# Monash-Connected-Autonomous-Vehicle/unsupervised-pseuso-LiDAR

Hardware: AMD Instinct MI355X
Metric: images/sec (fwd+bwd) KITTI 192x640 triplets, full training step (higher is better)
Workload: dtype f32; 1 GPU; BASELINE.json configs[1]: per-GPU batch=12, 192x640 KITTI-shaped triplets, ResNet-18 depth encoder + 6-DoF PoseNet, fp32 (the ResNet trunk's 3x3 stride-1 convolutions and their data gradients: fp32 contractions on split operands -- three bf16 planes per operand, six bf16-MFMA plane products, fp32 accumulation; every other launch: fp32 MFMA), one step = 2x depth fwd + pose fwd + warp/L1/smooth loss; global_batch=12, parallelism=dp1

## Files before the change

include/mcav_conv.h:

```cpp
#ifndef MCAV_CONV_H
#define MCAV_CONV_H

#include <stddef.h>
#include <stdint.h>

#ifdef __cplusplus
extern "C" {
#endif

#define MCAV_G_DIRECT 0
#define MCAV_G_SMALLC 1
#define MCAV_G_ADJ_REFLECT 2
#define MCAV_G_ADJ_STRIDE2 3

#define MCAV_PAD_ZERO 0
#define MCAV_PAD_REFLECT 1

#define MCAV_ACT_NONE 0
#define MCAV_ACT_RELU 1
#define MCAV_ACT_ELU 2
#define MCAV_ACT_SIGMOID 3

#define MCAV_DACT_AFTER_ADDEND 0x100

typedef struct mcav_igemm_desc {
    const float* x1;
    const float* x2;
    int B, Hs, Ws, C1, C2;
    int up1;
    const float* w;
    int kh, kw, Np, Kp;
    int mode, stride, sign, offset, pad_mode;
    float* y;
    int Hd, Wd, Cd, n_begin, n_count, y_choff;
    const float* bias;
    int act;
    const float* dact_aux;
    int dact;
    const float* addend;
    int pool;
    float* stats;
    int tile;
    int groups;
    const float* w_upmerge;
    int mma;
    const void* w16;
    const float* stats_x;
    const float* stats_mean;
    const float* stats_invstd;
    const float* w_stem;
    const float* x_planar[3];
    int planar_B;
    int planar_stack;
} mcav_igemm_desc;

int mcav_igemm_mtiles(const mcav_igemm_desc* d);
int mcav_igemm(const mcav_igemm_desc* d, void* stream);
int mcav_igemm_uses_bf16(const mcav_igemm_desc* d);

typedef struct mcav_wgrad_desc {
    const float* x1;
    const float* x2;
    int B, Hs, Ws, C1, C2, up1;
    int kh, kw, Kp;
    int mode, stride, sign, offset, pad_mode;
    const float* dy;
    int Hd, Wd, Cdy, dy_choff;
    int Cout, Cin;
    float* dw_oihw;
    int accumulate;
    float* dbias;
    int tile;
    int upm, Cin_total, ci_offset;
    int mma;
    const float* dy_bn_x;
    const float* dy_bn_gamma;
    const float* dy_bn_mean;
    const float* dy_bn_invstd;
    const float* dy_bn_sums;
    int dy_bn_groups;
    float dy_bn_inv_count;
    const float* x_planar[3];
    int planar_B;
    int planar_stack;
} mcav_wgrad_desc;

size_t mcav_wgrad_workspace_bytes(const mcav_wgrad_desc* d);
int mcav_wgrad_uses_bf16(const mcav_wgrad_desc* d);
int mcav_wgrad(const mcav_wgrad_desc* d, void* workspace, size_t workspace_bytes, void* stream);

typedef struct mcav_wgrad_reduce_item {
    const float* slab;
    float* pre;
    float* dw;
    float* dbias;
    unsigned long long elems;
    int splits, groups, per_group, Ktot, slabN, Kp, taps, Cout, Cin, ci_t, accumulate, upm, cin_total, ci_off;
    int pre_bx, red_gx, red_gy, pre_first, red_first, reserved;
} mcav_wgrad_reduce_item;
int mcav_wgrad_deferred(const mcav_wgrad_desc* d, void* workspace, size_t workspace_bytes, mcav_wgrad_reduce_item* item, void* stream);
int mcav_wgrad_reduce_plan(mcav_wgrad_reduce_item* items, int n, int* presum_blocks, int* reduce_blocks, size_t* lds_bytes);
int mcav_wgrad_reduce_multi(const mcav_wgrad_reduce_item* items_dev, int n, int presum_blocks, int reduce_blocks, size_t lds_bytes, void* stream);

int mcav_pack_weights(const float* w_oihw, int Cout, int Cin, int kh, int kw, int transposed, float* packed, int Np, int Kp,
                      void* stream);

int mcav_pack_weights_multi(const void* items_dev, int nitems, int nblocks, void* stream);
int mcav_f32_to_bf16(const float* src, void* dst_bf16, size_t n, void* stream);
int mcav_f32_to_bf16_planes(const float* src, void* dst_bf16, size_t n, void* stream);
int mcav_pack_weights_blocks(int taps, int transposed, int Np, int Kp);
int mcav_pack_stem_weights(const float* w_oihw, int Cout, int Cin, float* packed, void* stream);
int mcav_pack_weights_upmerge(const float* w_oihw, int Cout, int Cin, int C1, float* packed, int Np, void* stream);
int mcav_pack_weights_upmerge_adj(const float* w_oihw, int Cout, int Cin, int C1, float* packed, int Np, int Kp, void* stream);
int mcav_upsample_adj_fold(const float* tmp, int B, int Hl, int Wl, int C, const float* dact_aux, int dact, const float* addend, float* out,
                           void* stream);

int mcav_conv3x3r_c1_fwd(const float* x, int B, int H, int W, int C, const float* w_oihw, const float* bias, int act, float* y,
                         void* stream);
size_t mcav_conv3x3r_c1_bwd_workspace_bytes(int C);
int mcav_conv3x3r_c1_bwd(const float* x, int B, int H, int W, int C, const float* w_oihw, const float* dy, const float* y, int act,
                         int x_act, const float* addend, float* dx, float* dw_oihw, float* dbias, int accumulate, void* workspace,
                         size_t workspace_bytes, void* stream);

int mcav_kernel_timer_begin(void);
int mcav_kernel_timer_count(void);
int mcav_kernel_timer_end(float* ms, int capacity);

int mcav_nchw_to_nhwc(const float* src, int B, int C, int H, int W, float* dst, int Cp, int choff, void* stream);
int mcav_nhwc_to_nchw(const float* src, int B, int C, int H, int W, int Cp, int choff, float* dst, void* stream);
int mcav_nchw3_to_nhwc(const float* s0, const float* s1, const float* s2, int B, int C, int H, int W, float* dst, int Cp, void* stream);

int mcav_bn_finalize(const float* stats, int mtiles, int C, double count, const float* gamma, const float* beta, float eps,
                     float momentum, float* running_mean, float* running_var, float* scale, float* shift, float* save_mean,
                     float* save_invstd, int groups, void* workspace, size_t workspace_bytes, void* stream);
size_t mcav_bn_finalize_workspace_bytes(int mtiles, int C, int groups);
int mcav_bn_eval_coeffs(const float* gamma, const float* beta, const float* running_mean, const float* running_var, float eps, int C,
                        float* scale, float* shift, void* stream);
int mcav_bn_apply(const float* x, const float* scale, const float* shift, const float* residual, int act, size_t n_pix, int C, float* y,
                  size_t pix_per_group, void* stream);
size_t mcav_bn_bwd_workspace_bytes(size_t n_pix, int C, int groups);
int mcav_bn_bwd_reduce(const float* dy, const float* y_act, const float* x, const float* save_mean, const float* save_invstd, int relu,
                       size_t n_pix, int C, float* dgamma, float* dbeta, int accumulate, float* sums ,
                       int groups, void* workspace, size_t workspace_bytes, void* stream);
int mcav_bn_bwd_finalize(const float* partial, int nblk, int C, float* dgamma, float* dbeta, int accumulate, float* sums, int groups, void* stream);
int mcav_bn_bwd_apply(const float* dy, const float* y_act, const float* x, const float* gamma, const float* save_mean,
                      const float* save_invstd, const float* sums, int relu, size_t n_pix, int C, float* dx, float* dres,
                      int dres_accumulate, int groups, void* stream);

int mcav_maxpool3s2_fwd(const float* x, int B, int H, int W, int C, float* y, uint8_t* idx, void* stream);
int mcav_maxpool3s2_bwd(const float* dy, const uint8_t* idx, int B, int H, int W, int C, float* dx, int accumulate, void* stream);

int mcav_stem_bn_relu_pool_fwd(const float* x, const float* scale, const float* shift, int B, int H, int W, int C, int groups, float* y,
                               float* pooled, uint8_t* idx, void* stream);
int mcav_stem_pool_bn_bwd_reduce(float* dy, const float* dpooled, const uint8_t* idx, const float* x, const float* scale, const float* shift,
                                 const float* save_mean, const float* save_invstd, int B, int H, int W, int C, int groups, int store_dz,
                                 float* dgamma, float* dbeta, int accumulate, float* sums , void* workspace,
                                 size_t workspace_bytes, void* stream);
int mcav_stem_pool_bn_bwd_apply(const float* dy, const float* dpooled, const uint8_t* idx, const float* x, const float* scale,
                                const float* shift, const float* gamma, const float* save_mean, const float* save_invstd, const float* sums,
                                int B, int H, int W, int C, int groups, float* dx, void* stream);

int mcav_act_bwd(const float* dy, const float* y, int act, size_t n, float* dx, int accumulate, void* stream);
int mcav_act_bwd_strided(const float* dy, const float* y, int act, size_t n, float* dx, int stride, void* stream);
int mcav_add(const float* a, const float* b, size_t n, float* out, void* stream);
int mcav_spatial_mean(const float* x, int B, int n_pix, int C, float scale, float* out, void* stream);
int mcav_spatial_mean_bwd(const float* dout, int B, int n_pix, int C, float scale, float* dx, void* stream);

int mcav_copy_channels(const float* src, size_t n_pix, int Cs, int soff, float* dst, int Cd, int doff, int C, int accumulate, void* stream);
int mcav_resize_bilinear_fwd(const float* src, int B, int h, int w, float* dst, int H, int W, float scale_y, float scale_x, void* stream);
int mcav_resize_bilinear_bwd(const float* ddst, int B, int h, int w, float* dsrc, int H, int W, float scale_y, float scale_x, int accumulate,
                             void* stream);
int mcav_upsample_nearest2x(const float* src, size_t planes, int h, int w, float* dst, void* stream);
int mcav_upsample_nearest2x_bwd(const float* grad_out, size_t planes, int h, int w, float* grad_in, void* stream);
int mcav_affine(const float* x, float a, float b, size_t n, float* y, void* stream);
int mcav_mul(const float* a, const float* b, size_t n, float* y, void* stream);
size_t mcav_colsum_workspace_bytes(int C);
int mcav_colsum(const float* x, size_t n_pix, int C, float* out, int accumulate, void* workspace, size_t workspace_bytes, void* stream);

int mcav_adam_step(float* param, const float* grad, float* exp_avg, float* exp_avg_sq, size_t n, float lr, float beta1, float beta2,
                   float eps, int step, float grad_scale, void* stream);

int mcav_adam_step_dev(float* param, const float* grad, float* exp_avg, float* exp_avg_sq, size_t n, float beta1, float beta2, float eps,
                       float* state8, void* stream);

int mcav_event_create(void** event);
int mcav_event_destroy(void* event);
int mcav_event_record_external(void* event, void* stream);
int mcav_event_wait_external(void* event, void* stream);
int mcav_stream_wait_event(void* stream, void* event);

#ifdef __cplusplus
}
#endif
#endif
```

unsupervised-pseuso-lidar_amd/csrc/conv_bf16.hip:

```cpp
#include "conv_shared.h"
#include "kernel_timer.h"

namespace mcav {

typedef __bf16 bf16x8 __attribute__((ext_vector_type(8)));
typedef __bf16 bf16x4 __attribute__((ext_vector_type(4)));
typedef __bf16 bf16x2 __attribute__((ext_vector_type(2)));
typedef unsigned short u16;
typedef unsigned int u32x2 __attribute__((ext_vector_type(2)));

template <int BM_, int BN_, int WM_, int WN_, int MF_, int CK_>
struct BTile {
    static constexpr int BM = BM_, BN = BN_, WM = WM_, WN = WN_, MF = MF_;
    static constexpr int KD = CK_;
    static constexpr int LDH = CK_ + 8;
    static constexpr int LPRA = CK_ / 4;
    static constexpr int RPPA = 256 / LPRA;
    static constexpr int AROWS = BM / RPPA;
    static constexpr int LPRB = CK_ / 8;
    static constexpr int BVECS = (BN * LPRB + 255) / 256;
    static constexpr int WAVES_M = BM / WM, WAVES_N = BN / WN;
    static constexpr int TM = WM / MF, TN = WN / MF;
    static constexpr int ACC = MF == 32 ? 16 : 4;
    using AccT = typename std::conditional<MF_ == 32, f32x16, f32x4>::type;
// ... 262 lines not shown
            issue(ra, rb, ex);
            store(ra, rb, ex, B0{});
            if (T_total > 1) issue(ra, rb, ex);
        }
    } else {
        if (T_total > 0) {
            issue(ra, rb, ex);
            if (T_total > 1) issue(ra2, rb2, ex2);
            store(ra, rb, ex, B0{});
            if (T_total > 2) issue(ra, rb, ex);
        }
    }
    __syncthreads();
    if constexpr (NS == 1) {
        int t = 0;
        for (; t + 1 < T_total; t += 2) {
            store(ra, rb, ex, B1{});
            if (t + 2 < T_total) issue(ra, rb, ex);
            compute(B0{});
            __syncthreads();
            if (t + 2 < T_total) {
                store(ra, rb, ex, B0{});
                if (t + 3 < T_total) issue(ra, rb, ex);
            }
            compute(B1{});
            __syncthreads();
        }
        if (t < T_total) {
            compute(B0{});
            __syncthreads();
        }
    } else {
        for (int t = 0; t < T_total; t += 2) {
            compute(B0{});
            __syncthreads();
            if (t + 1 < T_total) {
                store(ra2, rb2, ex2, B0{});
                if (t + 3 < T_total) issue(ra2, rb2, ex2);
                __syncthreads();
                compute(B0{});
                __syncthreads();
                if (t + 2 < T_total) {
                    store(ra, rb, ex, B0{});
                    if (t + 4 < T_total) issue(ra, rb, ex);
                    __syncthreads();
                }
            }
        }
#pragma unroll
        for (int i = 0; i < T::TM; ++i)
#pragma unroll
            for (int j = 0; j < T::TN; ++j) acc[i][j] += mid[i][j] + low[i][j];
    }
    igemm_epilogue_lean<T>(p, acc, s_out, s_stat, tid, wm0, wn0, n0, mt);
}

__device__ __forceinline__ int patch_pixel(int R) {
    const int r = R & 31;
    const bool g0 = r < 4 || (r >= 12 && r < 16) || (r >= 20 && r < 28);
    const int idx = g0 ? (r < 4 ? r : (r < 16 ? r - 8 : r - 12)) : (r < 12 ? r - 4 : (r < 20 ? r - 8 : r - 16));
    return (R & ~31) + (g0 ? 0 : 16) + idx;
}

__device__ __forceinline__ int small_div(int n, float rcp_d) { return (int)(((float)n + 0.5f) * rcp_d); }

struct PatchGeo {
    int TH, TW, tiles_y, tiles_x;
    int tmb;
    int refl;
};

#ifndef MCAV_PATCH_DIAG
#define MCAV_PATCH_DIAG 0
#endif

template <int TMB>
struct PatchCfg {
    static constexpr int BM = 64 * TMB;
    static constexpr int PIX = TMB == 1 ? 110 : 180;
    static constexpr int NJ = (PIX + 31) / 32;
    using T = typename std::conditional<TMB == 1, BT64x64k32, BT128x64k32>::type;
};

template <int NS, int TMB, bool ADJ = false>
__global__ __launch_bounds__(256, 2) void conv3x3_patch_kernel(IgemmParams p, const u16* __restrict__ w16, PatchGeo geo) {
    using C = PatchCfg<TMB>;
    using T = typename C::T;
    constexpr int BM = C::BM, BN = 64, CKT = 32, LDH = 32, PATCH_PIX = C::PIX;
    constexpr int APL = PATCH_PIX * LDH, BPL = BN * LDH;
    extern __shared__ __attribute__((aligned(16))) unsigned char s_raw[];
    u16* const Ap = reinterpret_cast<u16*>(s_raw);
    u16* const Bs = Ap + NS * APL;
    unsigned* const s_out = reinterpret_cast<unsigned*>(Bs + 3 * NS * BPL);
    float (*const s_stat)[2][BN] = reinterpret_cast<float (*)[2][BN]>(Bs);
    static_assert(sizeof(u16) * BPL >= sizeof(float) * T::WAVES_M * 2 * BN, "statistics scratch fits a filter plane");

    const int tid = threadIdx.x, lane = tid & 63, wave = tid >> 6;
    const int lid = xcd_remap(blockIdx.x, gridDim.x);
    const int nt = lid % p.ntiles, mt = lid / p.ntiles;
    const int n0 = nt * BN;
    const GatherSrc& g = p.g;
    const int TH = geo.TH, TW = geo.TW, PW = TW + 2, PH = TH + 2;
    const int per_img = geo.tiles_y * geo.tiles_x;
    const float rcp_pw = 1.0f / (float)PW, rcp_tw = 1.0f / (float)TW;
    const int img = small_div(mt, 1.0f / (float)per_img), tr = mt - img * per_img;
    const int tyi = small_div(tr, 1.0f / (float)geo.tiles_x);
    const int ty0 = tyi * TH, tx0 = (tr - tyi * geo.tiles_x) * TW;
// ... 176 lines not shown
                    mid[t] = __builtin_amdgcn_mfma_f32_32x32x16_bf16(a[0], b[1], mid[t], 0, 0, 0);
                    low[t] = __builtin_amdgcn_mfma_f32_32x32x16_bf16(a[1], b[1], low[t], 0, 0, 0);
                }
            }
            __builtin_amdgcn_sched_barrier(0);
        }
    };

    constexpr bool TWO = TMB == 1;
    f32x4 ra[C::NJ], rb0[3][NS], rb1[TWO ? 3 : 1][NS];
    const int total = nchunks * 3;
    issueA(ra, 0);
    issueB(rb0, 0);
    storeA(ra);
    storeB(rb0);
    if (total > 1) issueB(rb0, 1);
    if constexpr (TWO) {
        if (total > 2) issueB(rb1, 2);
    }
    __syncthreads();
    int ky = 0, chunk = 0;
    constexpr int diag = MCAV_PATCH_DIAG;
    auto stage = [&](int s, auto& rb_next) {
        const bool more = chunk + 1 < nchunks;
        if (ky == 0 && more && !(diag & 4)) issueA(ra, chunk + 1);
        if (!(diag & 8)) compute(ky);
        if constexpr (ADJ) {
            if (has_y1 | has_yl | has_x1 | has_xl) extras(ky);
        }
        if (!(diag & 2)) __syncthreads();
        if (ky == 2 && more && !(diag & 4)) storeA(ra);
        if (s + 1 < total) {
            if (!(diag & 1)) {
                storeB(rb_next);
                if (s + (TWO ? 3 : 2) < total) issueB(rb_next, s + (TWO ? 3 : 2));
            }
            if (!(diag & 2)) __syncthreads();
        }
        if (++ky == 3) { ky = 0; ++chunk; }
    };
    if constexpr (TWO) {
        for (int s = 0; s < total; s += 2) {
            stage(s, rb0);
            if (s + 1 < total) stage(s + 1, rb1);
        }
    } else {
        for (int s = 0; s < total; ++s) stage(s, rb0);
    }
    if constexpr (NS > 1) {
#pragma unroll
        for (int t = 0; t < TMB; ++t) acc[t][0] += mid[t] + low[t];
    }
    if (diag & 16) return;
    igemm_epilogue_lean<T>(p, acc, s_out, s_stat, tid, wm0, wn0, n0, mt);
}

template <int NS, int TMB>
constexpr size_t patch_lds_bytes() { return sizeof(u16) * (size_t)NS * (PatchCfg<TMB>::PIX + 3 * 64) * 32 + sizeof(unsigned) * 64 * TMB; }

struct P3Tile {
    static constexpr int BM = 192, BN = 64, MF = 32, ACC = 16, TM = 1, TN = 1, WAVES_M = 6, WAVES_N = 2;
    using AccT = f32x16;
};
constexpr int P3_THREADS = 768, P3_SUBS = 3, P3_PIX = 110;
template <int NS> constexpr size_t patch3_lds_bytes() { return sizeof(u16) * (size_t)NS * (P3_SUBS * P3_PIX + 2 * 3 * 64) * 32 + sizeof(unsigned) * 192; }
#ifndef MCAV_PATCH3_DIAG
#define MCAV_PATCH3_DIAG 0
#endif

template <int NS, bool ADJ>
__global__ __launch_bounds__(P3_THREADS, 1) void conv3x3_patch3_kernel(IgemmParams p, const u16* __restrict__ w16, PatchGeo geo) {
    using T = P3Tile;
    constexpr int BN = 64, CKT = 32, LDH = 32, PIX = P3_PIX;
    constexpr int APL = PIX * LDH, BPL = BN * LDH;
    constexpr int ASUB = NS * APL, BSTAGE = 3 * NS * BPL;
    constexpr int diag = MCAV_PATCH3_DIAG;
    extern __shared__ __attribute__((aligned(16))) unsigned char s_raw[];
    u16* const Ap = reinterpret_cast<u16*>(s_raw);
    u16* const Bs = Ap + P3_SUBS * ASUB;
    unsigned* const s_out = reinterpret_cast<unsigned*>(Bs + 2 * BSTAGE);
    float (*const s_stat)[2][BN] = reinterpret_cast<float (*)[2][BN]>(Bs);
    static_assert(sizeof(u16) * BSTAGE >= sizeof(float) * T::WAVES_M * 2 * BN, "statistics scratch fits a ring stage");

    const int tid = threadIdx.x, lane = tid & 63, wave = __builtin_amdgcn_readfirstlane(tid >> 6);
    const int sub = wave >> 2, wm0 = sub * 64 + ((wave >> 1) & 1) * 32, wn0 = (wave & 1) * 32;
    const int lid = xcd_remap(blockIdx.x, gridDim.x);
    const int nt = lid % p.ntiles, mt = lid / p.ntiles;
    const int n0 = nt * BN;
    const GatherSrc& g = p.g;
    const int TH = geo.TH, TW = geo.TW, PW = TW + 2, PH = TH + 2;
    const int per_img = geo.tiles_y * geo.tiles_x, nblocks = g.B * per_img;
    const float rcp_pw = 1.0f / (float)PW, rcp_tw = 1.0f / (float)TW;
    int b_img[P3_SUBS], b_ty0[P3_SUBS], b_tx0[P3_SUBS];
#pragma unroll
    for (int sb = 0; sb < P3_SUBS; ++sb) {
        const int blk = mt * P3_SUBS + sb;
        const int img = blk / per_img, tr = blk - img * per_img, tyi = tr / geo.tiles_x;
        b_img[sb] = blk < nblocks ? img : -1;
        b_ty0[sb] = tyi * TH;
        b_tx0[sb] = (tr - tyi * geo.tiles_x) * TW;
    }
    auto pick = [&](const int (&v)[P3_SUBS], int sb) { return sb == 0 ? v[0] : (sb == 1 ? v[1] : v[2]); };

    if (tid < 192) {
        const int sb = tid >> 6;
        const int pix = patch_pixel(tid & 63);
        const int py = small_div(pix, rcp_tw), px = pix - py * TW;
// ... 134 lines not shown
        const int rsh = (fwd ? ky : 2 - ky) * PW + (fwd ? 0 : 2);
        const int dxr = fwd ? 1 : -1;
        bf16x8 fa[2][NS], fb[2][NS];
        auto load = [&](int i, bf16x8 (&a)[NS], bf16x8 (&b)[NS]) {
            const int kx = i >> 1, ks = i & 1;
            const u16* const bp = Bst + (ks ? b_lane1 : b_lane0) + kx * NS * BPL;
#pragma unroll
            for (int q = 0; q < NS; ++q) b[q] = *reinterpret_cast<const bf16x8*>(bp + q * BPL);
            const int row = prow + rsh + kx * dxr;
            const u16* const ap = Asub + row * LDH + (((2 * ks + fslot) ^ ((row >> 2) & 3)) * 8);
#pragma unroll
            for (int q = 0; q < NS; ++q) a[q] = *reinterpret_cast<const bf16x8*>(ap + q * APL);
        };
        load(0, fa[0], fb[0]);
#pragma unroll
        for (int i = 0; i < 6; ++i) {
            if (i + 1 < 6) load(i + 1, fa[(i + 1) & 1], fb[(i + 1) & 1]);
            __builtin_amdgcn_sched_barrier(0);
            if (!(diag & 8)) mma(fa[i & 1], fb[i & 1]);
            __builtin_amdgcn_sched_barrier(0);
        }
    };

    f32x4 ra[NJ], rbn[NS];
    const int total = nchunks * 3;
    issueA(ra, 0);
    issueB(rbn, 0);
    storeA(ra);
    storeB(rbn, 0);
    if (total > 1) issueB(rbn, 1);
    __syncthreads();
    int ky = 0, chunk = 0;
    for (int s = 0; s < total; ++s) {
        const bool more = chunk + 1 < nchunks;
        const u16* const Bst = Bs + (s & 1) * BSTAGE;
        if (ky == 0 && more && !(diag & 4)) issueA(ra, chunk + 1);
        compute(ky, Bst);
        if constexpr (ADJ) {
            if (has_y1 | has_yl | has_x1 | has_xl) extras(ky, Bst);
        }
        if (s + 1 < total && !(diag & 1)) {
            storeB(rbn, (s + 1) & 1);
            if (s + 2 < total) issueB(rbn, s + 2);
        }
        if (ky == 2 && more && !(diag & 4)) {
            __syncthreads();
            storeA(ra);
        }
        __syncthreads();
        if (++ky == 3) { ky = 0; ++chunk; }
    }
    if constexpr (NS > 1) acc[0][0] += mid + low;
    if (diag & 16) return;
    igemm_epilogue_lean<T>(p, acc, s_out, s_stat, tid, wm0, wn0, n0, mt);
}

#ifndef MCAV_PATCH2_DIAG
#define MCAV_PATCH2_DIAG 0
#endif

template <int SB, int BN_>
struct Patch2Cfg {
    static constexpr int BM = 64 * SB, BN = BN_;
    static constexpr int PIX = 110;
    static constexpr int VP = SB * PIX;
    static constexpr int NJ = (VP + 31) / 32;
    using T = typename std::conditional<SB == 4, BTile<256, BN_, 64, BN_, 32, 32>, BTile<128, BN_, 32, BN_, 32, 32>>::type;
};

template <int NS, int SB, int BN>
constexpr size_t patch2_lds_bytes() { return sizeof(u16) * (size_t)NS * (SB * 110 + 2 * 3 * BN) * 32 + sizeof(unsigned) * 64 * SB; }

template <int NS, int SB, int BN>
__global__ __launch_bounds__(256, BN == 32 ? 2 : 1) void conv3x3_patch2_kernel(IgemmParams p, const u16* __restrict__ w16, PatchGeo geo) {
    using C = Patch2Cfg<SB, BN>;
    using T = typename C::T;
    constexpr int BM = C::BM, CKT = 32, LDH = 32, PIX = C::PIX, TM = T::TM, TN = T::TN;
    constexpr int APL = PIX * LDH;
    constexpr int BPL = BN * LDH;
    constexpr int BSTAGE = 3 * NS * BPL;
    extern __shared__ __attribute__((aligned(16))) unsigned char s_raw[];
    u16* const Ap = reinterpret_cast<u16*>(s_raw);
    u16* const Bs = Ap + SB * NS * APL;
    unsigned* const s_out = reinterpret_cast<unsigned*>(Bs + 2 * BSTAGE);
    float (*const s_stat)[2][BN] = reinterpret_cast<float (*)[2][BN]>(Bs);
    static_assert(sizeof(u16) * BSTAGE >= sizeof(float) * T::WAVES_M * 2 * BN, "statistics scratch fits a filter stage");

    const int tid = threadIdx.x, lane = tid & 63, wave = tid >> 6;
    const int lid = xcd_remap(blockIdx.x, gridDim.x);
    const int nt = lid % p.ntiles, mt = lid / p.ntiles;
    const int n0 = nt * BN;
    const GatherSrc& g = p.g;
    const int TH = geo.TH, TW = geo.TW, PW = TW + 2, PH = TH + 2;
    const int per_img = geo.tiles_y * geo.tiles_x, nblk = g.B * per_img;

    __shared__ int s_pp[C::PIX];
    if (tid < PIX) {
        const int ppy = tid / PW;
        s_pp[tid] = tid < PH * PW ? (ppy << 8) | (tid - ppy * PW) : -1;
    }
    int sb_base[SB], sb_y0[SB], sb_x0[SB];
#pragma unroll
    for (int sb = 0; sb < SB; ++sb) {
        const int blk = mt * SB + sb;
        const int img = blk / per_img, tr = blk - img * per_img, tyi = tr / geo.tiles_x;
        sb_base[sb] = blk < nblk ? img : -1;
        sb_y0[sb] = tyi * TH;
// ... 1300 lines not shown
```

unsupervised-pseuso-lidar_amd/csrc/conv_gather.h:

```cpp
#pragma once
#include "mcav_common.h"
#include "../../include/mcav_conv.h"

namespace mcav {

typedef float f32x4 __attribute__((ext_vector_type(4)));
typedef float f32x16 __attribute__((ext_vector_type(16)));

constexpr int CK = 16;
constexpr int LDK = CK + 4;

struct GatherSrc {
    const float* x1;
    const float* x2;
    int B, Hs, Ws, C1, C2, up1;
    int mode, stride, sign, offset, pad_mode;
};

__device__ __forceinline__ int reflect_idx(int i, int n) {
    i = i < 0 ? -i : i;
    return i >= n ? 2 * n - 2 - i : i;
}

__device__ __forceinline__ f32x4 load_src4(const GatherSrc& g, int n, int sy, int sx, int c) {
// ... 23 lines not shown

__device__ __forceinline__ f32x4 gather4(const GatherSrc& g, int n, int dy, int dx, int ky, int kx, int c) {
    f32x4 z = {0.f, 0.f, 0.f, 0.f};
    if (g.mode == MCAV_G_DIRECT || g.mode == MCAV_G_SMALLC) {
        int sy = dy * g.stride + g.sign * ky + g.offset;
        int sx = dx * g.stride + g.sign * kx + g.offset;
        if (g.pad_mode == MCAV_PAD_REFLECT) {
            sy = reflect_idx(sy, g.Hs);
            sx = reflect_idx(sx, g.Ws);
        } else if ((unsigned)sy >= (unsigned)g.Hs || (unsigned)sx >= (unsigned)g.Ws) {
            return z;
        }
        return load_src4(g, n, sy, sx, c);
    }
    if (g.mode == MCAV_G_ADJ_REFLECT) {
        int ys[2], xs[2], ny = 0, nx = 0;
        const int sy = dy + 1 - ky, sx = dx + 1 - kx;
        if ((unsigned)sy < (unsigned)g.Hs) ys[ny++] = sy;
        if (dy == 1 && ky == 0) ys[ny++] = 0;
        if (dy == g.Hs - 2 && ky == 2) ys[ny++] = g.Hs - 1;
        if ((unsigned)sx < (unsigned)g.Ws) xs[nx++] = sx;
        if (dx == 1 && kx == 0) xs[nx++] = 0;
        if (dx == g.Ws - 2 && kx == 2) xs[nx++] = g.Ws - 1;
        for (int a = 0; a < ny; ++a)
            for (int b = 0; b < nx; ++b) z += load_src4(g, n, ys[a], xs[b], c);
        return z;
    }
    const int ty = dy + g.offset - ky, tx = dx + g.offset - kx;
    if (ty < 0 || tx < 0 || ((ty | tx) & 1)) return z;
    const int sy = ty >> 1, sx = tx >> 1;
    if (sy >= g.Hs || sx >= g.Ws) return z;
    return load_src4(g, n, sy, sx, c);
}

__device__ __forceinline__ int xcd_remap(int bid, int nwg) {
    const int q = nwg >> 3, r = nwg & 7, xcd = bid & 7;
    return (xcd < r ? xcd * (q + 1) : r * (q + 1) + (xcd - r) * q) + (bid >> 3);
}

struct IgemmParams {
    GatherSrc g;
    const float* w;
    int kh, kw, Kp, Kstride, taps;
    float* y;
    int Hd, Wd, Cd, n_begin, n_count, y_choff;
    const float* bias;
    int act;
    const float* dact_aux;
    int dact;
    const float* addend;
    int pool;
    float* stats;
    const float *stats_x, *stats_mean, *stats_invstd;
    int M;
    int Mc, McP;
    int groups;
    int mtiles, ntiles;
    int no_tab;
    const float* wm;
    int Np_all;
    int bm;
    int upm;
    int ksplit;
    float* kslab;
};

__device__ __forceinline__ float act_fwd(float v, int act) {
    if (act == MCAV_ACT_RELU) return v > 0.f ? v : 0.f;
    if (act == MCAV_ACT_ELU) return v > 0.f ? v : expm1f(v);
    if (act == MCAV_ACT_SIGMOID) return 1.0f / (1.0f + expf(-v));
    return v;
}

__device__ __forceinline__ float act_bwd(float y, int act) {
    if (act == MCAV_ACT_RELU) return y > 0.f ? 1.f : 0.f;
    if (act == MCAV_ACT_ELU) return y > 0.f ? 1.f : y + 1.f;
    if (act == MCAV_ACT_SIGMOID) return y * (1.f - y);
    return 1.f;
}

typedef unsigned int u32x4 __attribute__((ext_vector_type(4)));
constexpr unsigned OOB = 0x80000000u;

__device__ __forceinline__ __amdgpu_buffer_rsrc_t make_rsrc(const void* ptr, unsigned bytes) {
    return __builtin_amdgcn_make_buffer_rsrc(const_cast<void*>(ptr), 0, bytes, 0x00020000);
}

__device__ __forceinline__ f32x4 buf_load4(__amdgpu_buffer_rsrc_t r, unsigned byte_off) {
    return __builtin_bit_cast(f32x4, __builtin_amdgcn_raw_buffer_load_b128(r, (int)byte_off, 0, 0));
}

__device__ __forceinline__ f32x4 buf_load4s(__amdgpu_buffer_rsrc_t r, unsigned byte_off, int sbyte_off) {
    return __builtin_bit_cast(f32x4, __builtin_amdgcn_raw_buffer_load_b128(r, (int)byte_off, sbyte_off, 0));
}

__device__ __forceinline__ float buf_load1(__amdgpu_buffer_rsrc_t r, unsigned byte_off) {
    return __builtin_bit_cast(float, __builtin_amdgcn_raw_buffer_load_b32(r, (int)byte_off, 0, 0));
}

__device__ __forceinline__ void buf_store1(__amdgpu_buffer_rsrc_t r, unsigned byte_off, float v) {
    __builtin_amdgcn_raw_buffer_store_b32(__builtin_bit_cast(unsigned, v), r, (int)byte_off, 0, 0);
}

}
```

unsupervised-pseuso-lidar_amd/csrc/conv_igemm.hip:

```cpp
#include <stdlib.h>
#include <map>
#include <mutex>
#include <type_traits>
#include <utility>

#include "conv_shared.h"
#include "kernel_timer.h"

namespace mcav {

template <class T, int KIND>
__global__ __launch_bounds__(256) void igemm_kernel(IgemmParams p) {
    constexpr int BM = T::BM, BN = T::BN;
    constexpr int CK = T::KD;
    __shared__ __attribute__((aligned(16))) float As[2][BM][T::LD];
    __shared__ __attribute__((aligned(16))) float Bs[2][BN][T::LD];
    __shared__ int s_out[BM];
    __shared__ float s_stat[T::WAVES_M][2][BN];
    constexpr int MAXTAB = 9;
    __shared__ unsigned s_o1[KIND == K_GENERIC ? 1 : MAXTAB][KIND == K_GENERIC ? 1 : BM];
    __shared__ unsigned s_o2[KIND == K_GENERIC ? 1 : MAXTAB][KIND == K_GENERIC ? 1 : BM];
    __shared__ int s_rn[KIND == K_GENERIC ? 1 : BM], s_ry[KIND == K_GENERIC ? 1 : BM], s_rx[KIND == K_GENERIC ? 1 : BM];

    const int tid = threadIdx.x, lane = tid & 63, wave = tid >> 6;
// ... 215 lines not shown
#pragma unroll
            for (int ks = 0; ks < CK / 8; ++ks) {
                f32x4 a[T::TM], b[T::TN];
#pragma unroll
                for (int i = 0; i < T::TM; ++i) a[i] = *reinterpret_cast<const f32x4*>(&As[buf][wm0 + i * 32 + frow][ks * 8 + fk]);
#pragma unroll
                for (int j = 0; j < T::TN; ++j) b[j] = *reinterpret_cast<const f32x4*>(&Bs[buf][wn0 + j * 32 + frow][ks * 8 + fk]);
#pragma unroll
                for (int q = 0; q < 4; ++q)
#pragma unroll
                    for (int i = 0; i < T::TM; ++i)
#pragma unroll
                        for (int j = 0; j < T::TN; ++j)
                            acc[i][j] = __builtin_amdgcn_mfma_f32_32x32x2f32(a[i][q], b[j][q], acc[i][j], 0, 0, 0);
            }
        } else {
            const int frow = lane & 15, fk = (lane >> 4) * 4;
#pragma unroll
            for (int ks = 0; ks < CK / 16; ++ks) {
                f32x4 a[T::TM], b[T::TN];
#pragma unroll
                for (int i = 0; i < T::TM; ++i) a[i] = *reinterpret_cast<const f32x4*>(&As[buf][wm0 + i * 16 + frow][ks * 16 + fk]);
#pragma unroll
                for (int j = 0; j < T::TN; ++j) b[j] = *reinterpret_cast<const f32x4*>(&Bs[buf][wn0 + j * 16 + frow][ks * 16 + fk]);
#pragma unroll
                for (int q = 0; q < 4; ++q)
#pragma unroll
                    for (int i = 0; i < T::TM; ++i)
#pragma unroll
                        for (int j = 0; j < T::TN; ++j)
                            acc[i][j] = __builtin_amdgcn_mfma_f32_16x16x4f32(a[i][q], b[j][q], acc[i][j], 0, 0, 0);
            }
        }
    };

    f32x4 ra[T::AROWS], rb[T::BVECS];
    if (T_total > 0) {
        load_tile(ra, rb, true);
        store_tile(ra, rb, 0);
        if (T_total > 1) { advance(); load_tile(ra, rb, true); }
    }
    __syncthreads();
    for (int t = 0; t < T_total; ++t) {
        const int buf = t & 1;
        if (t + 1 < T_total) {
            store_tile(ra, rb, buf ^ 1);
            if (t + 2 < T_total) { advance(); load_tile(ra, rb, true); }
        }
        __builtin_amdgcn_sched_barrier(0);
        compute(buf);
        __builtin_amdgcn_sched_barrier(0);
        __syncthreads();
    }
    igemm_epilogue<T>(p, acc, s_out, s_stat, tid, wm0, wn0, n0, mt);
}


#ifndef MCAV_DIAG
#define MCAV_DIAG 0
#endif
#if MCAV_DIAG == 4
__device__ unsigned long long g_diag_stamps[8];
#define MCAV_STAMP_BEGIN() unsigned long long st_prev = __builtin_readcyclecounter()
#define MCAV_STAMP(i) do { __syncthreads(); if (threadIdx.x == 0) { const unsigned long long st_now = __builtin_readcyclecounter(); \
        atomicAdd(&g_diag_stamps[i], st_now - st_prev); if (i == 5) atomicAdd(&g_diag_stamps[0], 1ull); st_prev = st_now; } } while (0)
#else
#define MCAV_STAMP_BEGIN()
#define MCAV_STAMP(i)
#endif
#ifndef MCAV_IG_OCC
#define MCAV_IG_OCC 1
#endif
template <class T, int TK>
__global__ __launch_bounds__(256, (T::BM == 128 && T::BN == 64 && T::KD == 16 && TK != 1) ? 4
                                  : ((T::BM == 64 && T::BN == 64 && T::KD == 32 && TK == 0) ? MCAV_IG_OCC : 1)) void igemm_tab_kernel(IgemmParams p) {
    constexpr bool REFL = TK == 1, UPM = TK == 2;
    constexpr int BM = T::BM, BN = T::BN, CKT = T::KD;
    __shared__ __attribute__((aligned(16))) float As[2][BM][T::LD];
    __shared__ __attribute__((aligned(16))) float Bs[2][BN][T::LD];
    __shared__ __attribute__((aligned(16))) unsigned s_out[BM];
    float (*const s_stat)[2][BN] = reinterpret_cast<float (*)[2][BN]>(&As[1][0][0]);
    static_assert(sizeof(float) * BM * T::LD >= sizeof(float) * T::WAVES_M * 2 * BN, "statistics scratch fits one A buffer");
    extern __shared__ unsigned s_dyn[];
    unsigned* const s_o1 = s_dyn;
    unsigned* const s_o2 = s_dyn + (UPM ? 4 * BM : (p.g.C2 > 0 ? p.taps * BM : 0));
    int* const s_rn = reinterpret_cast<int*>(&As[0][0][0]);
    unsigned* const s_e0 = s_dyn + p.taps * BM;
    unsigned* const s_e1 = s_dyn + 2 * p.taps * BM;
    unsigned* const s_e2 = s_dyn + 3 * p.taps * BM;
    int* const s_ry = s_rn + BM;
    int* const s_rx = s_rn + 2 * BM;
    static_assert(2 * BM * T::LD >= 3 * BM, "row coordinates fit the A panel");
    __shared__ int s_tl[TAB_TAPS + 1];
    __shared__ int s_nt;

    const int tid = threadIdx.x, lane = tid & 63, wave = tid >> 6;
    MCAV_STAMP_BEGIN();
    const int lid = p.g.mode == MCAV_G_ADJ_STRIDE2 ? (int)blockIdx.x : xcd_remap(blockIdx.x, gridDim.x);
    const int per_split = p.mtiles * p.ntiles;
    const int ks = p.ksplit > 1 ? lid / per_split : 0, lrem = lid - ks * per_split;
    const int nt = lrem % p.ntiles, mt = lrem / p.ntiles;
    const int m0 = mt * BM, n0 = nt * BN;
    const GatherSrc& g = p.g;

    for (int r = tid; r < (MCAV_DIAG >= 5 ? 0 : BM); r += 256) {
        int n, dy, dx;
        const bool ok = decode_row(p, m0 + r, n, dy, dx);
// ... 363 lines not shown
                    else if constexpr (WHOLE_ISSUE && P == T::AROWS + T::BVECS) issue(ra, rb);
                    else piece(std::integral_constant<int, P>{}, nxt);
                });
                __builtin_amdgcn_sched_barrier(0);
            });
        });
        if constexpr (MCAV_DIAG < 3) __syncthreads();
    };
    MCAV_STAMP(1);
    int t = 0;
    using Yes = std::true_type;
    using No = std::false_type;
    if (T_total > 0) {
        if constexpr (REFL) {
            issue(ra, rb);
            store(ra, rb, B0{});
            if (T_total > 1) issue(ra, rb);
        } else if constexpr (MCAV_DIAG >= 6) {
#pragma unroll
            for (int j = 0; j < T::AROWS; ++j) ra[j] = f32x4{1.f, 1.f, 1.f, 1.f};
#pragma unroll
            for (int j = 0; j < T::BVECS; ++j) rb[j] = f32x4{1.f, 1.f, 1.f, 1.f};
            store(ra, rb, B0{});
        } else {
            f32x4 ra0[T::AROWS], rb0[T::BVECS];
            issue(ra0, rb0);
            if (T_total > 1) issue(ra, rb);
            store(ra0, rb0, B0{});
        }
    }
    __syncthreads();
    MCAV_STAMP(2);
    for (; t + 3 < T_total; t += 2) {
        step(B0{}, B1{}, Yes{}, Yes{});
        step(B1{}, B0{}, Yes{}, Yes{});
    }
    MCAV_STAMP(3);
    const int rest = T_total - t;
    if (rest == 3) {
        step(B0{}, B1{}, Yes{}, Yes{});
        step(B1{}, B0{}, Yes{}, No{});
        step(B0{}, B1{}, No{}, No{});
    } else if (rest == 2) {
        step(B0{}, B1{}, Yes{}, No{});
        step(B1{}, B0{}, No{}, No{});
    } else if (rest == 1) {
        step(B0{}, B1{}, No{}, No{});
    }
    MCAV_STAMP(4);
    if (p.ksplit > 1) {
        IgemmParams q = p;
        q.y = p.kslab + (size_t)ks * ((size_t)p.g.B * p.Hd * p.Wd * p.Cd);
        q.bias = nullptr; q.act = MCAV_ACT_NONE; q.dact_aux = nullptr; q.addend = nullptr; q.stats = nullptr; q.stats_x = nullptr;
        igemm_epilogue_lean<T>(q, acc, s_out, s_stat, tid, wm0, wn0, n0, mt);
    } else {
        igemm_epilogue_lean<T>(p, acc, s_out, s_stat, tid, wm0, wn0, n0, mt);
    }
    MCAV_STAMP(5);
}

template <class T, int KIND>
__global__ __launch_bounds__(256) void wgrad_kernel(WgradParams p) {
    constexpr int BM = T::BM, BN = T::BN;
    __shared__ __attribute__((aligned(16))) float Xs[2][KP][BM];
    __shared__ __attribute__((aligned(16))) float Ys[2][KP][BN];
    const int tid = threadIdx.x, lane = tid & 63, wave = tid >> 6;
    const int per_split = p.mtiles * p.ntiles;
    const int lid_ = xcd_remap(blockIdx.x, gridDim.x);
    const int split = lid_ / per_split, rem = lid_ - split * per_split;
    const int nt = rem % p.ntiles, mt = rem / p.ntiles;
    const int m0 = mt * BM, n0 = nt * BN;
    const GatherSrc& g = p.g;

    constexpr int ACOLS = BM / 4;
    constexpr int APIX = 256 / ACOLS;
    constexpr int APASS = KP / APIX;
    constexpr int CPW = ACOLS / 4;
    const int acol = wave * CPW + lane % CPW, apix = lane / CPW;
    const int kflat = m0 + acol * 4;
    int aky = -1, akx = 0, ac = 0;
    if (kflat < p.Ktot) {
        const int tap = kflat / p.Kp;
        ac = kflat - tap * p.Kp;
        aky = tap / p.kw; akx = tap - aky * p.kw;
        if (tap >= p.taps) aky = -1;
    }
    constexpr int BCOLS = BN / 4;
    constexpr int BPIX = 256 / BCOLS > KP ? KP : 256 / BCOLS;
    constexpr int BPASS = KP / BPIX;
    const int bcol = tid % BCOLS, bpix = tid / BCOLS;

    const int pix_begin = split * p.pix_per_split;
    const int pix_end = min(p.Mpix, pix_begin + p.pix_per_split);
    const int T_total = pix_end > pix_begin ? (pix_end - pix_begin + KP - 1) / KP : 0;

    int pn, py, px;
    {
        const int m = pix_begin + apix;
        pn = m / (p.Hd * p.Wd);
        const int r = m - pn * (p.Hd * p.Wd);
        py = r / p.Wd; px = r - py * p.Wd;
    }
    auto step_pix = [&](int& n, int& y, int& x, int by) {
        x += by;
        if constexpr (KIND == K_FAST) {
            const bool wx = x >= p.Wd;
            x = wx ? x - p.Wd : x;
            y += wx ? 1 : 0;
            const bool wy = y >= p.Hd;
// ... 786 lines not shown
inline int kstride_of(int taps, int Kp) { return round_up(taps * Kp, CK); }

inline int pick_tile(const mcav_igemm_desc* d, long M) {
    if (d->tile) return d->tile;
    if (d->n_count <= 16) return (M >= 256 * 64 && d->kh * d->kw <= 16) ? 4 : 6;
    if (d->n_count <= 32) return 7;
    if (d->mode == MCAV_G_ADJ_REFLECT && ((M + 127) / 128) * ((d->n_count + 63) / 64) >= 1024) return 2;
    if (d->mode != MCAV_G_SMALLC && ((M + 127) / 128) * ((d->n_count + 63) / 64) >= 1024) return 1;
    const long t64 = ((M + 63) / 64) * ((d->n_count + 63) / 64);
    if (d->mode != MCAV_G_SMALLC && d->Kp % 32 == 0 && (t64 <= 128 || (t64 > 256 && t64 < 512))) return 12;
    if (d->mode != MCAV_G_SMALLC && d->Kp % 32 == 0) return 10;
    const long t128x64 = ((M + 127) / 128) * ((d->n_count + 63) / 64);
    return t128x64 >= 1024 ? 1 : 2;
}

void tile_dims(int id, int& BM, int& BN) {
    switch (id) {
        case 1: BM = 128; BN = 64; break;
        case 2: BM = 64; BN = 64; break;
        case 3: BM = 256; BN = 32; break;
        case 4: BM = 256; BN = 16; break;
        case 5: BM = 128; BN = 128; break;
        case 7: BM = 128; BN = 32; break;
        case 8: BM = 128; BN = 64; break;
        case 9: BM = 128; BN = 128; break;
        case 10: BM = 64; BN = 64; break;
        case 11: BM = 64; BN = 64; break;
        case 12: BM = 32; BN = 64; break;
        default: BM = 64; BN = 16; break;
    }
}

bool fill_params(const mcav_igemm_desc* d, IgemmParams& p, int& tile) {
    if (!d || !d->x1 || !d->w || !d->y) return false;
    if (d->B <= 0 || d->Hs <= 0 || d->Ws <= 0 || d->Hd <= 0 || d->Wd <= 0 || d->C1 <= 0 || d->C2 < 0) return false;
    if (d->C2 > 0 && !d->x2) return false;
    if (d->kh <= 0 || d->kw <= 0 || d->Np <= 0 || d->Kp <= 0 || d->kh * d->kw > 64) return false;
    if (d->n_begin < 0 || d->n_count <= 0 || d->n_begin + d->n_count > d->Np) return false;
    if (d->mode == MCAV_G_SMALLC) { if (d->Kp != 4 || d->C1 != 4 || d->C2 != 0) return false; }
    else if (d->Kp % CK != 0 || d->Kp < d->C1 + d->C2) return false;
    if (d->C2 > 0 && (d->C1 % 4 != 0)) return false;
    if (d->mode == MCAV_G_ADJ_REFLECT && (d->kh != 3 || d->kw != 3 || d->Hs != d->Hd || d->Ws != d->Wd || d->Hs < 2 || d->Ws < 2)) return false;
    if (d->pad_mode == MCAV_PAD_REFLECT && (d->Hs < 2 || d->Ws < 2)) return false;
    if (d->up1 && ((d->Hs & 1) || (d->Ws & 1))) return false;
    if (d->pool && ((d->Hd & 1) || (d->Wd & 1) || d->mode == MCAV_G_ADJ_STRIDE2)) return false;
    if (d->pool && d->stats) return false;
    p.g.x1 = d->x1; p.g.x2 = d->x2; p.g.B = d->B; p.g.Hs = d->Hs; p.g.Ws = d->Ws; p.g.C1 = d->C1; p.g.C2 = d->C2; p.g.up1 = d->up1;
    p.g.mode = d->mode; p.g.stride = d->stride; p.g.sign = d->sign; p.g.offset = d->offset; p.g.pad_mode = d->pad_mode;
    p.w = d->w; p.kh = d->kh; p.kw = d->kw; p.Kp = d->Kp; p.taps = d->kh * d->kw; p.Kstride = kstride_of(p.taps, d->Kp);
    p.y = d->y; p.Hd = d->Hd; p.Wd = d->Wd; p.Cd = d->Cd; p.n_begin = d->n_begin; p.n_count = d->n_count; p.y_choff = d->y_choff;
    p.bias = d->bias; p.act = d->act; p.dact_aux = d->dact_aux; p.dact = d->dact; p.addend = d->addend; p.pool = d->pool; p.stats = d->stats;
    if (d->stats_x && (!d->stats || !d->stats_mean || !d->stats_invstd || d->pool || d->y_choff != 0 || d->n_begin != 0 || d->n_count != d->Cd)) return false;
    p.stats_x = d->stats ? d->stats_x : nullptr; p.stats_mean = d->stats_mean; p.stats_invstd = d->stats_invstd;
    const long Mlin = (long)d->B * d->Hd * d->Wd;
    if ((long)d->B * d->Hs * d->Ws * (d->C1 > d->C2 ? d->C1 : d->C2) * 4 >= 0x7fffffffL) return false;
    if ((long)d->Np * kstride_of(d->kh * d->kw, d->Kp) * 4 >= 0x7fffffffL) return false;
    p.no_tab = (d->tile >> 8) & 1;
    p.ksplit = 1; p.kslab = nullptr;
    p.wm = d->w_upmerge; p.Np_all = d->Np; p.upm = 0;
    tile = pick_tile(d, Mlin) & 0xff;
    if (tile == 0) { mcav_igemm_desc dd = *d; dd.tile = 0; tile = pick_tile(&dd, Mlin); }
    if (((tile >= 8 && tile <= 10) || tile == 12) && (d->mode == MCAV_G_SMALLC || d->Kp % 32 != 0)) return false;
    if (tile == 11 && (d->mode == MCAV_G_SMALLC || d->Kp % 64 != 0)) return false;
    int BM, BN;
    tile_dims(tile, BM, BN);
    p.groups = d->groups > 1 ? d->groups : 1;
    if (p.groups > 1) {
        if ((d->mode != MCAV_G_DIRECT && d->mode != MCAV_G_SMALLC) || d->pool || d->B % p.groups != 0) return false;
        p.Mc = (int)(Mlin / p.groups);
        p.McP = round_up(p.Mc, BM);
        p.M = p.groups * p.McP;
    } else if (d->mode == MCAV_G_ADJ_STRIDE2) {
        p.Mc = d->B * ((d->Hd + 1) / 2) * ((d->Wd + 1) / 2);
        p.McP = round_up(p.Mc, BM);
        p.M = 4 * p.McP;
    } else {
        p.Mc = 0; p.McP = 1;
        if (Mlin > 0x7fffffffL) return false;
        p.M = (int)Mlin;
        const int ck = (tile >= 8 && tile <= 10) || tile == 12 ? 32 : (tile == 11 ? 64 : 16);
        if (d->w_upmerge && d->mode == MCAV_G_DIRECT && d->kh == 3 && d->kw == 3 && d->stride == 1 && d->sign == 1 && d->offset == -1 &&
            d->pad_mode == MCAV_PAD_REFLECT && d->up1 == 1 && d->C2 > 0 && !(d->Hd & 1) && !(d->Wd & 1) && d->Hd == d->Hs && d->Wd == d->Ws &&
            !d->pool && !d->stats && d->C1 % ck == 0 && d->C2 % ck == 0 && d->C1 + d->C2 == d->Kp && (d->C1 & 3) == 0 && !p.no_tab &&
            (long)4 * d->Np * 4 * d->C1 * 4 < 0x7fffffffL) {
            p.upm = 1;
            p.bm = BM;
            p.Mc = d->B * (d->Hd / 2) * (d->Wd / 2);
            p.McP = round_up(p.Mc, BM);
            p.M = 4 * p.McP;
        }
    }
    p.mtiles = (p.M + BM - 1) / BM;
    p.ntiles = (d->n_count + BN - 1) / BN;
    return true;
}

__global__ __launch_bounds__(256) void splitk_finish_kernel(const float* __restrict__ slab, int splits, size_t n, int Cd, float* __restrict__ y,
                                                            const float* __restrict__ bias, int n_begin, int act, const float* __restrict__ dact_aux,
                                                            int dact, const float* __restrict__ addend) {
    for (size_t i = (size_t)blockIdx.x * 256 + threadIdx.x; i < n; i += (size_t)gridDim.x * 256) {
        float v = 0.f;
        for (int k = 0; k < splits; ++k) v += slab[(size_t)k * n + i];
        if (bias) v += bias[n_begin + (int)(i % (size_t)Cd)];
        v = act_fwd(v, act);
        if (dact_aux && !(dact & MCAV_DACT_AFTER_ADDEND)) v *= act_bwd(dact_aux[i], dact & 0xff);
        if (addend) v += addend[i];
// ... 41 lines not shown
            if (ksp > 8) ksp = 8;
            if (ksp > ktiles / 4) ksp = ktiles / 4;
            if (ksp >= 2) {
                float* slab = ksplit_slab(s, (size_t)p.g.B * p.Hd * p.Wd * p.Cd * 4 * ksp);
                if (slab) { p.ksplit = ksp; p.kslab = slab; }
            }
        }
    }
    const int grid = p.mtiles * p.ntiles * p.ksplit;
    const size_t tab_bytes = sizeof(unsigned) * (size_t)p.taps * T::BM * (p.g.C2 > 0 ? 2 : 1);
    const size_t refl_bytes = sizeof(unsigned) * (size_t)p.taps * T::BM * 4;
    if (p.upm) timed_launch(igemm_tab_kernel<T, 2>, grid, dim3(256), sizeof(unsigned) * 13 * T::BM, s, p);
    else if (tab) timed_launch(igemm_tab_kernel<T, 0>, grid, dim3(256), tab_bytes, s, p);
    else if (tab_refl) timed_launch(igemm_tab_kernel<T, 1>, grid, dim3(256), refl_bytes, s, p);
    else if (fast_mode && c4ok) timed_launch(igemm_kernel<T, K_FAST>, grid, dim3(256), 0, s, p);
    else if (p.g.mode == MCAV_G_ADJ_REFLECT && c4ok && p.g.C2 == 0) timed_launch(igemm_kernel<T, K_REFLADJ>, grid, dim3(256), 0, s, p);
    else timed_launch(igemm_kernel<T, K_GENERIC>, grid, dim3(256), 0, s, p);
    if (p.ksplit > 1) {
        const size_t n = (size_t)p.g.B * p.Hd * p.Wd * p.Cd;
        const int blocks = (int)((n + 255) / 256 < 2048 ? (n + 255) / 256 : 2048);
        timed_launch(splitk_finish_kernel, blocks, dim3(256), 0, s, (const float*)p.kslab, p.ksplit, n, p.Cd, p.y, p.bias, p.n_begin, p.act, p.dact_aux,
                     p.dact, p.addend);
    }
}

}

using namespace mcav;

int mcav_bf16_igemm_mtiles(const mcav_igemm_desc* d);
int mcav_patch_f32_mtiles(const mcav_igemm_desc* d);
bool mcav_try_patch_f32(const mcav_igemm_desc* d, hipStream_t s);
int mcav_stem_mtiles(const mcav_igemm_desc* d);

int mcav_stem_planar_igemm(const mcav_igemm_desc* d);

MCAV_EXPORT int mcav_igemm_mtiles(const mcav_igemm_desc* d) {
    IgemmParams p;
    int tile;
    const int planar = mcav_stem_planar_igemm(d);
    if (planar < 0) return MCAV_E_INVALID;
    mcav_igemm_desc dp;
    if (planar) { dp = *d; if (!dp.x1) dp.x1 = d->x_planar[0]; d = &dp; }
    if (!fill_params(d, p, tile)) return MCAV_E_INVALID;
    if (const int st = mcav_stem_mtiles(d)) return st;
    if (const int pt = mcav_patch_f32_mtiles(d)) return pt;
    if (d->mma != 0) {
        const int mt = mcav_bf16_igemm_mtiles(d);
        if (mt > 0) return mt;
    }
    return p.mtiles;
}

bool mcav_try_halo(const mcav_igemm_desc* d, hipStream_t s);
int mcav_bf16_igemm(const mcav_igemm_desc* d, hipStream_t s);
bool mcav_try_stem(const mcav_igemm_desc* d, const mcav::IgemmParams& p, hipStream_t s);
int mcav_stem_mtiles(const mcav_igemm_desc* d);
int mcav_stem_planar_igemm(const mcav_igemm_desc* d);
bool mcav_bf16_wgrad_plan(const mcav_wgrad_desc* d, mcav::WgradPlan& pl);
void mcav_bf16_wgrad_launch(const mcav::WgradParams& p, hipStream_t s);

MCAV_EXPORT int mcav_igemm(const mcav_igemm_desc* d, void* stream) {
    IgemmParams p;
    int tile;
    const int planar = mcav_stem_planar_igemm(d);
    if (planar < 0) return MCAV_E_INVALID;
    mcav_igemm_desc dp;
    if (planar) { dp = *d; if (!dp.x1) dp.x1 = d->x_planar[0]; d = &dp; }
    if (!fill_params(d, p, tile)) return MCAV_E_INVALID;
    hipStream_t s = as_stream(stream);
    if (planar) return mcav_try_stem(d, p, s) ? launch_status() : MCAV_E_INVALID;
    if (mcav_try_halo(d, s)) return launch_status();
    if (mcav_try_stem(d, p, s)) return launch_status();
    if (mcav_try_patch_f32(d, s)) return launch_status();
    if (d->mma != 0) {
        const int rc = mcav_bf16_igemm(d, s);
        if (rc != 1) return rc;
    }
    switch (tile) {
        case 1: launch_igemm<Tile128x64>(p, s); break;
        case 2: launch_igemm<Tile64x64>(p, s); break;
        case 3: launch_igemm<Tile256x32>(p, s); break;
        case 4: launch_igemm<Tile256x16>(p, s); break;
        case 5: launch_igemm<Tile128x128>(p, s); break;
        case 6: launch_igemm<Tile64x16>(p, s); break;
        case 7: launch_igemm<Tile128x32>(p, s); break;
        case 8: launch_igemm<Tile128x64k32>(p, s); break;
        case 9: launch_igemm<Tile128x128k32>(p, s); break;
        case 10: launch_igemm<Tile64x64k32>(p, s); break;
        case 11: launch_igemm<Tile64x64k64>(p, s); break;
        case 12: launch_igemm<Tile32x64k32>(p, s); break;
        default: return MCAV_E_INVALID;
    }
    return launch_status();
}

namespace mcav {

}
int mcav_stem_wgrad_splits(const mcav_wgrad_desc* d);
int mcav_stem_planar_wgrad(const mcav_wgrad_desc* d);
int mcav_stem_wgrad_bn(const mcav_wgrad_desc* d);
void mcav_stem_wgrad_launch(const mcav_wgrad_desc* d, float* slab, int Ktot, int slabN, int splits, hipStream_t s);
int mcav_halo_wgrad_splits(const mcav_wgrad_desc* d);
void mcav_halo_wgrad_launch(const mcav_wgrad_desc* d, float* slab, int slabN, int splits, hipStream_t s);
namespace mcav {

bool plan_wgrad(const mcav_wgrad_desc* d, WgradPlan& pl) {
    if (!d || !d->x1 || !d->dy || !d->dw_oihw) return false;
    if (d->B <= 0 || d->Hs <= 0 || d->Ws <= 0 || d->Hd <= 0 || d->Wd <= 0 || d->C1 <= 0 || d->C2 < 0 || d->Cout <= 0 || d->Cin <= 0) return false;
    if (d->C2 > 0 && (!d->x2 || d->C1 % 4 != 0)) return false;
    if (d->mode != MCAV_G_DIRECT && d->mode != MCAV_G_SMALLC) return false;
    if (d->mode == MCAV_G_SMALLC && (d->Kp != 4 || d->C1 != 4 || d->C2 != 0)) return false;
    if (d->mode == MCAV_G_DIRECT && (d->Kp % CK != 0 || d->Kp < d->C1 + d->C2)) return false;
    if (d->Cin > d->Kp) return false;
    WgradParams& p = pl.p;
    p.g.x1 = d->x1; p.g.x2 = d->x2; p.g.B = d->B; p.g.Hs = d->Hs; p.g.Ws = d->Ws; p.g.C1 = d->C1; p.g.C2 = d->C2; p.g.up1 = d->up1;
    p.g.mode = d->mode; p.g.stride = d->stride; p.g.sign = d->sign; p.g.offset = d->offset; p.g.pad_mode = d->pad_mode;
    p.kh = d->kh; p.kw = d->kw; p.Kp = d->Kp; p.taps = d->kh * d->kw; p.Ktot = p.taps * d->Kp;
    p.dy = d->dy; p.Hd = d->Hd; p.Wd = d->Wd; p.Cdy = d->Cdy; p.dy_choff = d->dy_choff; p.Cout = d->Cout;
    p.CoutLoad = round_up(d->Cout, 4) <= d->Cdy - d->dy_choff ? round_up(d->Cout, 4) : d->Cout;
    const long M = (long)d->B * d->Hd * d->Wd;
    if (M > 0x7fffffffL) return false;
// ... 295 lines not shown
```

unsupervised-pseuso-lidar_amd/csrc/conv_shared.h:

```cpp
#pragma once
#include <stdlib.h>
#include <type_traits>
#include <utility>

#include "conv_gather.h"

namespace mcav {

template <int BM_, int BN_, int WM_, int WN_, int MF_, int CK_ = 16>
struct Tile {
    static constexpr int BM = BM_, BN = BN_, WM = WM_, WN = WN_, MF = MF_;
    static constexpr int KD = CK_;
    static constexpr int LD = CK_ + 4;
    static constexpr int LPR = CK_ / 4;
    static constexpr int RPP = 256 / LPR;
    static constexpr int WAVES_M = BM / WM, WAVES_N = BN / WN;
    static constexpr int TM = WM / MF, TN = WN / MF;
    static constexpr int ACC = MF == 32 ? 16 : 4;
    using AccT = typename std::conditional<MF_ == 32, f32x16, f32x4>::type;
    static constexpr int AROWS = BM / RPP;
    static constexpr int BVECS = (BN * LPR + 255) / 256;
    static_assert(WAVES_M * WAVES_N == 4, "4 wavefronts per workgroup");
    static_assert(BM % RPP == 0, "BM multiple of the rows per pass");
};
// ... 18 lines not shown

__device__ __forceinline__ bool decode_row(const IgemmParams& p, int m, int& n, int& dy, int& dx) {
    if (p.g.mode == MCAV_G_ADJ_STRIDE2) {
        const int blk = m / p.McP, r = m - blk * p.McP, cls = 3 - blk;
        if (r >= p.Mc) return false;
        const int Hc = (p.Hd + 1) >> 1, Wc = (p.Wd + 1) >> 1;
        n = r / (Hc * Wc);
        const int q = r - n * (Hc * Wc);
        const int y2 = q / Wc, x2 = q - y2 * Wc;
        dy = 2 * y2 + (cls >> 1);
        dx = 2 * x2 + (cls & 1);
        return dy < p.Hd && dx < p.Wd;
    }
    if (m >= p.M) return false;
    if (p.upm) {
        const int blk = m / p.bm, cls = blk & 3, r = (blk >> 2) * p.bm + (m - blk * p.bm);
        if (r >= p.Mc) return false;
        const int Hc = p.Hd >> 1, Wc = p.Wd >> 1;
        n = r / (Hc * Wc);
        const int q = r - n * (Hc * Wc);
        const int y2 = q / Wc, x2 = q - y2 * Wc;
        dy = 2 * y2 + (cls >> 1);
        dx = 2 * x2 + (cls & 1);
        return true;
    }
    if (p.groups > 1) {
        const int grp = m / p.McP, r = m - grp * p.McP;
        if (r >= p.Mc) return false;
        const int hw = p.Hd * p.Wd, ng = r / hw, q = r - ng * hw;
        n = grp * (p.g.B / p.groups) + ng;
        dy = q / p.Wd;
        dx = q - dy * p.Wd;
        return true;
    }
    if (p.pool) {
        const int blk = m >> 2, q = m & 3;
        const int Hh = p.Hd >> 1, Wh = p.Wd >> 1;
        n = blk / (Hh * Wh);
        const int r = blk - n * (Hh * Wh);
        const int y2 = r / Wh, x2 = r - y2 * Wh;
        dy = 2 * y2 + (q >> 1);
        dx = 2 * x2 + (q & 1);
        return true;
    }
    n = m / (p.Hd * p.Wd);
    const int r = m - n * (p.Hd * p.Wd);
    dy = r / p.Wd;
    dx = r - dy * p.Wd;
    return true;
}

enum { K_FAST = 0, K_REFLADJ = 1, K_GENERIC = 2 };

template <class T>
__device__ __forceinline__ void igemm_epilogue(const IgemmParams& p, typename T::AccT (&acc)[T::TM][T::TN], const int* s_out,
                                               float (*s_stat)[2][T::BN], int tid, int wm0, int wn0, int n0, int mt) {
    constexpr int BN = T::BN;
    const int lane = tid & 63, wave = tid >> 6;
    constexpr int MF = T::MF;
    const int ccol = lane & (MF - 1);
    float ssum[T::TN], ssq[T::TN];
#pragma unroll
    for (int j = 0; j < T::TN; ++j) { ssum[j] = 0.f; ssq[j] = 0.f; }
#pragma unroll
    for (int i = 0; i < T::TM; ++i)
#pragma unroll
        for (int j = 0; j < T::TN; ++j) {
            const int nl = n0 + wn0 + j * MF + ccol;
            const bool ncol = nl < p.n_count;
            const float bv = (p.bias && ncol) ? p.bias[p.n_begin + nl] : 0.f;
#pragma unroll
            for (int q = 0; q < T::ACC / 4; ++q) {
                const int rbase = wm0 + i * MF + (MF == 32 ? 8 * q + 4 * (lane >> 5) : 4 * (lane >> 4));
                float v[4];
#pragma unroll
                for (int e = 0; e < 4; ++e) v[e] = act_fwd(acc[i][j][4 * q + e] + bv, p.act);
                if (p.pool) {
                    const int o = s_out[rbase];
                    if (o >= 0 && ncol) {
                        float s = (v[0] + v[1]) + (v[2] + v[3]);
                        const size_t off = (size_t)o * p.Cd + p.y_choff + nl;
                        if (p.dact_aux && !(p.dact & MCAV_DACT_AFTER_ADDEND)) s *= act_bwd(p.dact_aux[off], p.dact & 0xff);
                        if (p.addend) s += p.addend[off];
                        if (p.dact_aux && (p.dact & MCAV_DACT_AFTER_ADDEND)) s *= act_bwd(p.dact_aux[off], p.dact & 0xff);
                        p.y[off] = s;
                    }
                } else {
#pragma unroll
                    for (int e = 0; e < 4; ++e) {
                        const int o = s_out[rbase + e];
                        if (o >= 0 && ncol) {
                            float s = v[e];
                            const size_t off = (size_t)o * p.Cd + p.y_choff + nl;
                            if (p.dact_aux && !(p.dact & MCAV_DACT_AFTER_ADDEND)) s *= act_bwd(p.dact_aux[off], p.dact & 0xff);
                            if (p.addend) s += p.addend[off];
                            if (p.dact_aux && (p.dact & MCAV_DACT_AFTER_ADDEND)) s *= act_bwd(p.dact_aux[off], p.dact & 0xff);
                            p.y[off] = s;
                            ssum[j] += s;
                            if (p.stats_x) {
                                const int gi = (mt / (p.mtiles / p.groups)) * p.n_count + nl;
                                ssq[j] += s * ((p.stats_x[off] - p.stats_mean[gi]) * p.stats_invstd[gi]);
                            } else {
                                ssq[j] += s * s;
                            }
                        }
                    }
                }
            }
        }
    if (p.stats) {
#pragma unroll
        for (int j = 0; j < T::TN; ++j) {
            if (MF == 32) {
                ssum[j] += __shfl_xor(ssum[j], 32, 64);
                ssq[j] += __shfl_xor(ssq[j], 32, 64);
            } else {
                ssum[j] += __shfl_xor(ssum[j], 16, 64); ssq[j] += __shfl_xor(ssq[j], 16, 64);
                ssum[j] += __shfl_xor(ssum[j], 32, 64); ssq[j] += __shfl_xor(ssq[j], 32, 64);
            }
            if (lane < MF) {
                s_stat[wave / T::WAVES_N][0][wn0 + j * MF + lane] = ssum[j];
                s_stat[wave / T::WAVES_N][1][wn0 + j * MF + lane] = ssq[j];
            }
        }
        __syncthreads();
        for (int e = tid; e < 2 * BN; e += 256) {
            const int which = e / BN, col = e - which * BN;
            if (n0 + col < p.n_count) {
                float s = 0.f;
#pragma unroll
                for (int wmi = 0; wmi < T::WAVES_M; ++wmi) s += s_stat[wmi][which][col];
                p.stats[((size_t)mt * 2 + which) * p.n_count + n0 + col] = s;
            }
        }
    }
}

template <class T>
__device__ __forceinline__ void igemm_epilogue_lean(const IgemmParams& p, typename T::AccT (&acc)[T::TM][T::TN], const unsigned* s_outb,
                                                    float (*s_stat)[2][T::BN], int tid, int wm0, int wn0, int n0, int mt) {
    constexpr int BN = T::BN, MF = T::MF, NQ = T::ACC / 4;
    const int lane = tid & 63, wave = tid >> 6;
    const int ccol = lane & (MF - 1);
    const unsigned ybytes = (unsigned)((size_t)p.g.B * (p.pool ? (p.Hd >> 1) * (p.Wd >> 1) : p.Hd * p.Wd) * p.Cd * 4);
    const __amdgpu_buffer_rsrc_t ry = make_rsrc(p.y, ybytes);
    const __amdgpu_buffer_rsrc_t rx = make_rsrc(p.dact_aux ? p.dact_aux : p.y, ybytes);
    const __amdgpu_buffer_rsrc_t rad = make_rsrc(p.addend ? p.addend : p.y, ybytes);
    const __amdgpu_buffer_rsrc_t rsx = make_rsrc(p.stats_x ? p.stats_x : p.y, ybytes);
    const int sgrp = p.stats_x ? (mt / (p.mtiles / p.groups)) * p.n_count : 0;
    float ssum[T::TN], ssq[T::TN];
#pragma unroll
    for (int j = 0; j < T::TN; ++j) { ssum[j] = 0.f; ssq[j] = 0.f; }
#pragma unroll
    for (int i = 0; i < T::TM; ++i)
#pragma unroll
        for (int j = 0; j < T::TN; ++j) {
            __builtin_amdgcn_sched_barrier(0);
            const int nl = n0 + wn0 + j * MF + ccol;
            if (nl < p.n_count) {
                const float bv = p.bias ? p.bias[p.n_begin + nl] : 0.f;
                const unsigned colb = (unsigned)(p.y_choff + nl) * 4u;
                u32x4 ro[NQ];
#pragma unroll
                for (int q = 0; q < NQ; ++q) {
                    const int rbase = wm0 + i * MF + (MF == 32 ? 8 * q + 4 * (lane >> 5) : 4 * (lane >> 4));
                    ro[q] = *reinterpret_cast<const u32x4*>(&s_outb[rbase]);
                }
                if (p.pool) {
                    float aux[NQ], add[NQ];
                    if (p.dact_aux) {
#pragma unroll
                        for (int q = 0; q < NQ; ++q) aux[q] = buf_load1(rx, ro[q].x + colb);
                    }
                    if (p.addend) {
#pragma unroll
                        for (int q = 0; q < NQ; ++q) add[q] = buf_load1(rad, ro[q].x + colb);
                    }
#pragma unroll
                    for (int q = 0; q < NQ; ++q) {
                        float v[4];
#pragma unroll
                        for (int e = 0; e < 4; ++e) v[e] = act_fwd(acc[i][j][4 * q + e] + bv, p.act);
                        float s = (v[0] + v[1]) + (v[2] + v[3]);
                        if (p.dact_aux && !(p.dact & MCAV_DACT_AFTER_ADDEND)) s *= act_bwd(aux[q], p.dact & 0xff);
                        if (p.addend) s += add[q];
                        if (p.dact_aux && (p.dact & MCAV_DACT_AFTER_ADDEND)) s *= act_bwd(aux[q], p.dact & 0xff);
                        buf_store1(ry, ro[q].x + colb, s);
                    }
                } else {
                    constexpr int QH = NQ >= 2 ? NQ / 2 : 1;
#pragma unroll
// ... 14 lines not shown
#pragma unroll
                                for (int e = 0; e < 4; ++e) aux[4 * q + e] = buf_load1(rx, ro[q0 + q][e] + colb);
                        }
                        if (p.addend) {
#pragma unroll
                            for (int q = 0; q < QH; ++q)
#pragma unroll
                                for (int e = 0; e < 4; ++e) add[4 * q + e] = buf_load1(rad, ro[q0 + q][e] + colb);
                        }
#pragma unroll
                        for (int q = 0; q < QH; ++q)
#pragma unroll
                            for (int e = 0; e < 4; ++e) {
                                float s = acc[i][j][4 * (q0 + q) + e] + bv;
                                if (p.act == MCAV_ACT_RELU) s = fmaxf(s, 0.f);
                                else if (p.act != MCAV_ACT_NONE) s = act_fwd(s, p.act);
                                if (p.dact_aux && !(p.dact & MCAV_DACT_AFTER_ADDEND)) s *= act_bwd(aux[4 * q + e], p.dact & 0xff);
                                if (p.addend) s += add[4 * q + e];
                                if (p.dact_aux && (p.dact & MCAV_DACT_AFTER_ADDEND)) s *= act_bwd(aux[4 * q + e], p.dact & 0xff);
                                buf_store1(ry, ro[q0 + q][e] + colb, s);
                                if (p.stats) {
                                    const float sv = ro[q0 + q][e] != OOB ? s : 0.f;
                                    ssum[j] += sv;
                                    ssq[j] += p.stats_x ? sv * ((xs[4 * q + e] - smu) * sis) : sv * sv;
                                }
                            }
                        __builtin_amdgcn_sched_barrier(0);
                    }
                }
            }
        }
    if (p.stats) {
#pragma unroll
        for (int j = 0; j < T::TN; ++j) {
            if (MF == 32) {
                ssum[j] += __shfl_xor(ssum[j], 32, 64);
                ssq[j] += __shfl_xor(ssq[j], 32, 64);
            } else {
                ssum[j] += __shfl_xor(ssum[j], 16, 64); ssq[j] += __shfl_xor(ssq[j], 16, 64);
                ssum[j] += __shfl_xor(ssum[j], 32, 64); ssq[j] += __shfl_xor(ssq[j], 32, 64);
            }
            if (lane < MF) {
                s_stat[wave / T::WAVES_N][0][wn0 + j * MF + lane] = ssum[j];
                s_stat[wave / T::WAVES_N][1][wn0 + j * MF + lane] = ssq[j];
            }
        }
        __syncthreads();
        for (int e = tid; e < 2 * BN; e += 256) {
            const int which = e / BN, col = e - which * BN;
            if (n0 + col < p.n_count) {
                float s = 0.f;
#pragma unroll
                for (int wmi = 0; wmi < T::WAVES_M; ++wmi) s += s_stat[wmi][which][col];
                p.stats[((size_t)mt * 2 + which) * p.n_count + n0 + col] = s;
            }
        }
    }
}

constexpr int TAB_TAPS = 32;
constexpr int WG_TABCAP = 2048;

struct WgradParams {
    GatherSrc g;
    int kh, kw, Kp, taps, Ktot;
    const float* dy;
    int Hd, Wd, Cdy, dy_choff, Cout;
    int CoutLoad;
    int Mpix;
    int splits, pix_per_split;
    int mtiles, ntiles;
    float* slab;
    int slabN;
    int want_bias;
    int tab_cht_log2;
    int upm;
    int Hf, Wf;
    int split_planes;
    int patch, pTH, pTW, ptiles_y, ptiles_x, prefl, pnblocks, pbps, pct_co, pnarrow;
};

constexpr int KP = 32;

struct WgradPlan {
    WgradParams p;
    int tile;
    bool use_tab;
    bool use_halo;
    bool use_stem;
    size_t slab_bytes, pre_bytes;
    int ci_t, groups, per_group;
};


bool fill_params(const mcav_igemm_desc* d, IgemmParams& p, int& tile);
bool plan_wgrad(const mcav_wgrad_desc* d, WgradPlan& pl);
void tile_dims(int id, int& BM, int& BN);

}
```

unsupervised-pseuso-lidar_amd/csrc/conv_stem.hip:

```cpp
#include "conv_shared.h"
#include "bn_bwd_formula.h"
#include "kernel_timer.h"

namespace mcav {

constexpr int ST_TW = 32;
constexpr int ST_PC = 36;

template <int C_, int CP_, int N_, int TH_>
struct StemCfg {
    static constexpr int C = C_, CP = CP_, N = N_, TH = TH_;
    static constexpr int PR = 2 * TH + 5;
    static constexpr int KS = C * 7 * 4;
    static constexpr int TM = TH / 4, TN = N >= 32 ? N / 32 : 1;
    static constexpr int NW = N;
    static constexpr int LD4 = (C + 3) / 4;
    using Epi = Tile<TH * 32, (N >= 32 ? N : 32), TM * 32, (N >= 32 ? N : 32), 32, 16>;
};
using StemDepth = StemCfg<3, 4, 64, 8>;
using StemPose = StemCfg<9, 16, 16, 4>;

struct StemPlanar {
    const float* src[3];
    int Bp;
// ... 162 lines not shown
    issue(blockIdx.x);
    for (int mt = blockIdx.x; mt < ntiles; mt += gridDim.x) {
        const int b = mt / per_img, tr = mt - b * per_img;
        const int ty = tr / tiles_x, tx = tr - ty * tiles_x;
        const int oy0 = ty * TH, ox0 = tx * ST_TW;
        __syncthreads();
        if (tid < TH * 32) {
            const int r = tid, oy = oy0 + (r >> 5), ox = ox0 + (r & 31);
            s_out[r] = (oy < p.Hd && ox < p.Wd) ? (unsigned)((b * p.Hd + oy) * p.Wd + ox) * (unsigned)(p.Cd * 4) : OOB;
        }
#pragma unroll
        for (int j = 0; j < PN; ++j) {
            const int i = tid + 256 * j;
            const int row = i / (2 * ST_PC), col = i - row * (2 * ST_PC);
            if (i < PR * 2 * ST_PC) {
#pragma unroll
                for (int c = 0; c < C; ++c) {
                    if constexpr (kPlanar) sP[c][row][col & 1][col >> 1] = pq[j][c];
                    else sP[c][row][col & 1][col >> 1] = pv[j][c >> 2][c & 3];
                }
            }
        }
        __syncthreads();
        issue(mt + gridDim.x);

        f32x16 acc[TM][TN];
#pragma unroll
        for (int i = 0; i < TM; ++i)
#pragma unroll
            for (int j = 0; j < TN; ++j)
#pragma unroll
                for (int r = 0; r < 16; ++r) acc[i][j][r] = 0.f;
        float fa[2][TM], fb[2][TN];
        auto rd = [&](auto sc) {
            constexpr int ks = decltype(sc)::value, kxp = ks & 3, cky = ks >> 2, ky = cky % 7, c = cky / 7, sl = ks & 1;
#pragma unroll
            for (int i = 0; i < TM; ++i) fa[sl][i] = pa[(c * PR + ky + 2 * i) * 2 * ST_PC + kxp];
#pragma unroll
            for (int j = 0; j < TN; ++j) fb[sl][j] = pb[ks * 2 * NW + 32 * j];
        };
        rd(std::integral_constant<int, 0>{});
        static_for<KS>([&](auto sc) {
            constexpr int ks = decltype(sc)::value, sl = ks & 1;
            if constexpr (ks + 1 < KS) rd(std::integral_constant<int, ks + 1>{});
            __builtin_amdgcn_sched_barrier(0);
#pragma unroll
            for (int i = 0; i < TM; ++i)
#pragma unroll
                for (int j = 0; j < TN; ++j) acc[i][j] = __builtin_amdgcn_mfma_f32_32x32x2f32(fa[sl][i], fb[sl][j], acc[i][j], 0, 0, 0);
            __builtin_amdgcn_sched_barrier(0);
        });
        __syncthreads();
        if constexpr (kWide) stem_epilogue_wide<E>(p, acc, s_out, s_stat, tid, wave * TM * 32, mt);
        else igemm_epilogue_lean<E>(p, acc, s_out, s_stat, tid, wave * TM * 32, 0, 0, mt);
    }
}

typedef __bf16 st_bf16x8 __attribute__((ext_vector_type(8)));
typedef __bf16 st_bf16x4 __attribute__((ext_vector_type(4)));
typedef unsigned short st_u16;
typedef unsigned int st_u32x2 __attribute__((ext_vector_type(2)));
constexpr int SS_TH = 8, SS_PR = 2 * SS_TH + 5, SS_PCOL = 72, SS_PROW = SS_PCOL * 4;
constexpr int SS_K = 224, SS_WROW = 232;
constexpr int SS_PPL = SS_PR * SS_PROW, SS_WPL = 64 * SS_WROW;
#ifndef MCAV_SS_DIAG
#define MCAV_SS_DIAG 0
#endif
constexpr int SS_DIAG = MCAV_SS_DIAG;
constexpr size_t stem_split_lds_bytes() { return sizeof(st_u16) * 3 * (size_t)(SS_PPL + SS_WPL) + sizeof(unsigned) * SS_TH * 32; }

__device__ __forceinline__ void st_split3(f32x4 v, st_u32x2& h, st_u32x2& m, st_u32x2& l) {
    const st_bf16x4 hb = __builtin_convertvector(v, st_bf16x4);
    const f32x4 r1 = v - __builtin_convertvector(hb, f32x4);
    const st_bf16x4 mb = __builtin_convertvector(r1, st_bf16x4);
    const f32x4 r2 = r1 - __builtin_convertvector(mb, f32x4);
    const st_bf16x4 lb = __builtin_convertvector(r2, st_bf16x4);
    h = __builtin_bit_cast(st_u32x2, hb); m = __builtin_bit_cast(st_u32x2, mb); l = __builtin_bit_cast(st_u32x2, lb);
}

template <bool kPlanar = false>
__global__ __launch_bounds__(256, 1) void stem7x7s2_split_fwd_kernel(IgemmParams p, const float* __restrict__ wk, int tiles_x, int tiles_y, StemPlanar pl) {
    using S = StemDepth;
    using E = typename S::Epi;
    constexpr int TM = S::TM, TN = S::TN, TH = S::TH;
    static_assert(TH == SS_TH && TM == 2 && TN == 2, "8 output rows per tile, 2 x 2 tiles per wavefront");
    extern __shared__ __attribute__((aligned(16))) unsigned char s_raw[];
    st_u16* const sP = reinterpret_cast<st_u16*>(s_raw);
    st_u16* const sW = sP + 3 * SS_PPL;
    unsigned* const s_out = reinterpret_cast<unsigned*>(sW + 3 * SS_WPL);
    float (*const s_stat)[2][E::BN] = reinterpret_cast<float (*)[2][E::BN]>(sP);

    const int tid = threadIdx.x, lane = tid & 63, wave = tid >> 6;
    const int per_img = tiles_x * tiles_y, ntiles = p.g.B * per_img;
    const GatherSrc& g = p.g;
    const __amdgpu_buffer_rsrc_t rsx = make_rsrc(g.x1, (unsigned)((size_t)g.B * g.Hs * g.Ws * S::CP * 4));

    constexpr int WN = 64 * SS_K / 256;
    float wv[WN];
#pragma unroll
    for (int j = 0; j < WN; ++j) {
        const int e = tid + 256 * j, co = e & 63, k = e >> 6, ky = k >> 5, kx = (k >> 2) & 7, c = k & 3;
        wv[j] = c < 3 ? wk[((c * 7 + ky) * 8 + kx) * 64 + co] : 0.f;
    }
#pragma unroll
    for (int j = 0; j < WN; ++j) {
        const int e = tid + 256 * j, co = e & 63, k = e >> 6;
        const float v = wv[j];
// ... 49 lines not shown
                *reinterpret_cast<st_u32x2*>(sP + i * 4) = hh;
                *reinterpret_cast<st_u32x2*>(sP + SS_PPL + i * 4) = mm;
                *reinterpret_cast<st_u32x2*>(sP + 2 * SS_PPL + i * 4) = ll;
            }
        }
        __syncthreads();
        issue(mt + gridDim.x);

        f32x16 acc[TM][TN], mid[TM][TN], low[TM][TN];
#pragma unroll
        for (int i = 0; i < TM; ++i)
#pragma unroll
            for (int j = 0; j < TN; ++j)
#pragma unroll
                for (int r = 0; r < 16; ++r) { acc[i][j][r] = 0.f; mid[i][j][r] = 0.f; low[i][j][r] = 0.f; }
        st_bf16x8 fa[2][TM][3], fb[2][TN][3];
        auto rd = [&](auto sc) {
            constexpr int ks = decltype(sc)::value, ky = ks >> 1, kh = ks & 1, sl = ks & 1;
#pragma unroll
            for (int i = 0; i < TM; ++i)
#pragma unroll
                for (int q = 0; q < 3; ++q) fa[sl][i][q] = *reinterpret_cast<const st_bf16x8*>(pa + q * SS_PPL + (2 * i + ky) * SS_PROW + 16 * kh);
#pragma unroll
            for (int j = 0; j < TN; ++j)
#pragma unroll
                for (int q = 0; q < 3; ++q) fb[sl][j][q] = *reinterpret_cast<const st_bf16x8*>(pb + q * SS_WPL + 32 * j * SS_WROW + 32 * ky + 16 * kh);
        };
        rd(std::integral_constant<int, 0>{});
        static_for<14>([&](auto sc) {
            constexpr int ks = decltype(sc)::value, sl = ks & 1;
            if constexpr (ks + 1 < 14) rd(std::integral_constant<int, ks + 1>{});
            __builtin_amdgcn_sched_barrier(0);
#pragma unroll
            for (int i = 0; i < TM; ++i)
#pragma unroll
                for (int j = 0; j < TN; ++j) {
                    const st_bf16x8(&a)[3] = fa[sl][i];
                    const st_bf16x8(&bq)[3] = fb[sl][j];
                    if (SS_DIAG & 1) continue;
                    low[i][j] = __builtin_amdgcn_mfma_f32_32x32x16_bf16(a[2], bq[0], low[i][j], 0, 0, 0);
                    mid[i][j] = __builtin_amdgcn_mfma_f32_32x32x16_bf16(a[1], bq[0], mid[i][j], 0, 0, 0);
                    acc[i][j] = __builtin_amdgcn_mfma_f32_32x32x16_bf16(a[0], bq[0], acc[i][j], 0, 0, 0);
                    low[i][j] = __builtin_amdgcn_mfma_f32_32x32x16_bf16(a[0], bq[2], low[i][j], 0, 0, 0);
                    mid[i][j] = __builtin_amdgcn_mfma_f32_32x32x16_bf16(a[0], bq[1], mid[i][j], 0, 0, 0);
                    low[i][j] = __builtin_amdgcn_mfma_f32_32x32x16_bf16(a[1], bq[1], low[i][j], 0, 0, 0);
                }
            __builtin_amdgcn_sched_barrier(0);
        });
#pragma unroll
        for (int i = 0; i < TM; ++i)
#pragma unroll
            for (int j = 0; j < TN; ++j) acc[i][j] += mid[i][j] + low[i][j];
        __syncthreads();
        if (!(SS_DIAG & 2)) igemm_epilogue_lean<E>(p, acc, s_out, s_stat, tid, wave * TM * 32, 0, 0, mt);
    }
}

__global__ void pack_stem_weights_kernel(const float* __restrict__ w, float* __restrict__ out, int C, int N) {
    const int i = blockIdx.x * blockDim.x + threadIdx.x;
    if (i >= C * 56 * N) return;
    const int n = i % N, k = i / N;
    const int hh = k & 1, j = (k >> 1) & 3, cky = k >> 3, ky = cky % 7, c = cky / 7;
    const int kx = 2 * j + hh;
    out[i] = kx < 7 ? w[((n * C + c) * 7 + ky) * 7 + kx] : 0.f;
}

constexpr int SW_TH = 4;
constexpr int SW_PR = 2 * SW_TH + 5;

struct StemWgradBn {
    const float* x;
    const float* gamma;
    const float* mean;
    const float* invstd;
    const float* sums;
    int groups;
    float inv_count;
};

template <int C, int CP, int N, int KP, bool kBN = false, bool kPlanar = false>
__global__ __launch_bounds__(256) void stem7x7s2_wgrad_kernel(const float* __restrict__ x4, const float* __restrict__ dy, int B, int Hs, int Ws,
                                                              int Hd, int Wd, int Cdy, int dy_choff, float* __restrict__ slab, int Ktot, int slabN,
                                                              int want_bias, StemWgradBn bn, StemPlanar pl) {
    constexpr int KS = C * 7 * 4, KT = (2 * KS + 31) / 32;
    constexpr int NSPLIT = N >= 64 ? 2 : 1, WPN = 4 / NSPLIT, MT = (KT + WPN - 1) / WPN;
    constexpr int LD4 = (C + 3) / 4, N4 = N / 4;
    __shared__ __attribute__((aligned(16))) float sP[C][SW_PR][2][ST_PC];
    __shared__ __attribute__((aligned(16))) float sDY[SW_TH * ST_TW][N];
    const int tid = threadIdx.x, lane = tid & 63, wave = tid >> 6;
    const int tiles_x = (Wd + ST_TW - 1) / ST_TW, tiles_y = (Hd + SW_TH - 1) / SW_TH;
    const int ntiles = B * tiles_x * tiles_y;
    const int i = lane & 31, h = lane >> 5;
    const int nt = NSPLIT == 2 ? wave & 1 : 0, mt0 = MT * (NSPLIT == 2 ? wave >> 1 : wave);
    int koff[MT];
#pragma unroll
    for (int m = 0; m < MT; ++m) {
        const int k = (mt0 + m) * 32 + i;
        const int par = k & 1, kxp = (k >> 1) & 3, cky = k >> 3, ky = cky % 7, c = cky / 7;
        koff[m] = k < 2 * KS ? ((c * SW_PR + ky) * 2 + par) * ST_PC + kxp + h : 0;
    }
    const float* const pP = &sP[0][0][0][0];
    const float* const pD = &sDY[h][nt * 32 + (N >= 32 ? i : i & (N - 1))];
    f32x16 acc[MT];
#pragma unroll
    for (int m = 0; m < MT; ++m)
#pragma unroll
        for (int r = 0; r < 16; ++r) acc[m][r] = 0.f;
// ... 272 lines not shown
```

unsupervised-pseuso-lidar_amd/csrc/nn_ops.hip:

```cpp
#include "conv_gather.h"
#include "bn_bwd_formula.h"

namespace mcav {

inline int grid_for(size_t work_items, int per_block = 256, int cap = 4096) {
    size_t b = (work_items + per_block - 1) / per_block;
    if (b < 1) b = 1;
    return (int)(b < (size_t)cap ? b : (size_t)cap);
}

__global__ void nchw_to_nhwc_kernel(const float* src, int B, int C, int H, int W, float* dst, int Cp, int choff) {
    const size_t plane = (size_t)H * W, total = (size_t)B * plane;
    for (size_t i = (size_t)blockIdx.x * blockDim.x + threadIdx.x; i < total; i += (size_t)gridDim.x * blockDim.x) {
        const size_t b = i / plane, pix = i - b * plane;
        for (int c = 0; c < C; ++c) dst[i * Cp + choff + c] = src[(b * C + c) * plane + pix];
    }
}

__global__ __launch_bounds__(256) void nchw_to_nhwc4_kernel(const float* src, int B, int C, int H, int W, float* dst) {
    const size_t plane = (size_t)H * W, total = (size_t)B * plane;
    for (size_t i = (size_t)blockIdx.x * blockDim.x + threadIdx.x; i < total; i += (size_t)gridDim.x * blockDim.x) {
        const size_t b = i / plane, pix = i - b * plane;
        f32x4 v = *reinterpret_cast<const f32x4*>(dst + i * 4);
        const float* s0 = src + (b * C) * plane + pix;
// ... 262 lines not shown
                                                              int groups) {
    __shared__ double s1[FIN_SL][32], s2[FIN_SL][32];
    const int cl = threadIdx.x & 31, slice = threadIdx.x >> 5, c = blockIdx.x * 32 + cl;
    double ta = 0.0, tb = 0.0;
    for (int g = 0; g < groups; ++g) {
        const float* pg = part + (size_t)g * nblk * 2 * C;
        double a = 0.0, b = 0.0;
        if (c < C) {
            int k = slice;
            for (; k + 7 * FIN_SL < nblk; k += 8 * FIN_SL) {
                float va[8], vb[8];
#pragma unroll
                for (int u = 0; u < 8; ++u) {
                    va[u] = pg[(size_t)(k + u * FIN_SL) * 2 * C + c];
                    vb[u] = pg[(size_t)(k + u * FIN_SL) * 2 * C + C + c];
                }
#pragma unroll
                for (int u = 0; u < 8; ++u) { a += (double)va[u]; b += (double)vb[u]; }
            }
            for (; k < nblk; k += FIN_SL) {
                a += (double)pg[(size_t)k * 2 * C + c];
                b += (double)pg[(size_t)k * 2 * C + C + c];
            }
        }
        s1[slice][cl] = a; s2[slice][cl] = b;
        __syncthreads();
        if (slice == 0 && c < C) {
            for (int k = 1; k < FIN_SL; ++k) { a += s1[k][cl]; b += s2[k][cl]; }
            sums[(size_t)g * 2 * C + c] = (float)a;
            sums[(size_t)g * 2 * C + C + c] = (float)b;
            ta += a; tb += b;
        }
        __syncthreads();
    }
    if (slice == 0 && c < C) {
        if (dbeta) dbeta[c] = accumulate ? dbeta[c] + (float)ta : (float)ta;
        if (dgamma) dgamma[c] = accumulate ? dgamma[c] + (float)tb : (float)tb;
    }
}

__global__ __launch_bounds__(256) void bn_bwd_apply_kernel(const f32x4* dy, const f32x4* yact, const f32x4* x, const f32x4* gamma, const f32x4* mean,
                                                           const f32x4* invstd, const f32x4* sums, int relu, size_t n4, int C4, float inv_count,
                                                           f32x4* dx, f32x4* dres, int dres_acc, size_t group4) {
    for (size_t i = (size_t)blockIdx.x * blockDim.x + threadIdx.x; i < n4; i += (size_t)gridDim.x * blockDim.x) {
        const int c = (int)(i % C4), grp = (int)(i / group4);
        f32x4 g = dy[i];
        if (relu) g = relu_mask(g, yact[i]);
        if (dres) dres[i] = dres_acc ? dres[i] + g : g;
        const f32x4 is = invstd[grp * C4 + c];
        const f32x4* sg = sums + (size_t)grp * 2 * C4;
        f32x4 gi, t2;
        bn_bwd_dx_coeffs(gamma[c], is, sg[C4 + c], inv_count, gi, t2);
        dx[i] = bn_bwd_dx(g, x[i], mean[grp * C4 + c], is, gi, sg[c], inv_count, t2);
    }
}

__global__ __launch_bounds__(256) void maxpool_fwd_kernel(const float* x, int B, int H, int W, int C, int Ho, int Wo, float* y, uint8_t* idx) {
    const int C4 = C >> 2;
    const size_t total = (size_t)B * Ho * Wo * C4;
    for (size_t i = (size_t)blockIdx.x * blockDim.x + threadIdx.x; i < total; i += (size_t)gridDim.x * blockDim.x) {
        const int c = (int)(i % C4);
        size_t r = i / C4;
        const int ox = (int)(r % Wo); r /= Wo;
        const int oy = (int)(r % Ho);
        const int b = (int)(r / Ho);
        const float ninf = -__builtin_huge_valf();
        f32x4 best = {ninf, ninf, ninf, ninf};
        int bi[4] = {0, 0, 0, 0};
        bool first[4] = {true, true, true, true};
#pragma unroll
        for (int ky = 0; ky < 3; ++ky) {
            const int iy = oy * 2 - 1 + ky;
            if ((unsigned)iy >= (unsigned)H) continue;
#pragma unroll
            for (int kx = 0; kx < 3; ++kx) {
                const int ix = ox * 2 - 1 + kx;
                if ((unsigned)ix >= (unsigned)W) continue;
                const f32x4 v = *reinterpret_cast<const f32x4*>(x + ((size_t)(b * H + iy) * W + ix) * C + c * 4);
#pragma unroll
                for (int e = 0; e < 4; ++e) {
                    if (first[e] || v[e] > best[e] || v[e] != v[e]) { best[e] = v[e]; bi[e] = ky * 3 + kx; first[e] = false; }
                }
            }
        }
        *reinterpret_cast<f32x4*>(y + i * 4) = best;
        uchar4 o;
        o.x = (uint8_t)bi[0]; o.y = (uint8_t)bi[1]; o.z = (uint8_t)bi[2]; o.w = (uint8_t)bi[3];
        *reinterpret_cast<uchar4*>(idx + i * 4) = o;
    }
}

__global__ __launch_bounds__(256) void maxpool_bwd_kernel(const float* dy, const uint8_t* idx, int B, int H, int W, int C, int Ho, int Wo, float* dx, int accumulate) {
    const int C4 = C >> 2;
    const size_t total = (size_t)B * H * W * C4;
    for (size_t i = (size_t)blockIdx.x * blockDim.x + threadIdx.x; i < total; i += (size_t)gridDim.x * blockDim.x) {
        const int c = (int)(i % C4);
        size_t r = i / C4;
        const int ix = (int)(r % W); r /= W;
        const int iy = (int)(r % H);
        const int b = (int)(r / H);
        f32x4 g = {0.f, 0.f, 0.f, 0.f};
        const int oy_lo = iy >> 1, oy_hi = (iy + 1) >> 1;
        const int ox_lo = ix >> 1, ox_hi = (ix + 1) >> 1;
        for (int oy = oy_lo; oy <= oy_hi; ++oy) {
            if (oy >= Ho) continue;
            const int ky = iy - (oy * 2 - 1);
// ... 160 lines not shown
    bn_apply_kernel<<<grid_for(n4), 256, 0, as_stream(stream)>>>((const f32x4*)x, (const f32x4*)scale, (const f32x4*)shift, (const f32x4*)residual,
                                                                 act == MCAV_ACT_RELU, n4, C / 4, (f32x4*)y,
                                                                 (pix_per_group ? pix_per_group : n_pix) * (size_t)(C / 4));
    return launch_status();
}

MCAV_EXPORT size_t mcav_bn_bwd_workspace_bytes(size_t n_pix, int C, int groups) {
    (void)n_pix;
    if (groups < 1) groups = 1;
    return C > 0 ? align_up(sizeof(float) * 2 * (size_t)C * BNR_BLOCKS * groups, 256) : 0;
}

MCAV_EXPORT int mcav_bn_bwd_reduce(const float* dy, const float* y_act, const float* x, const float* save_mean, const float* save_invstd, int relu,
                                   size_t n_pix, int C, float* dgamma, float* dbeta, int accumulate, float* sums, int groups, void* workspace,
                                   size_t workspace_bytes, void* stream) {
    if (groups < 1) groups = 1;
    if (!dy || !x || !save_mean || !save_invstd || !sums || !workspace || C <= 0 || (C & 3) || n_pix == 0 || n_pix % groups) return MCAV_E_INVALID;
    if (relu && !y_act) return MCAV_E_INVALID;
    const int C4 = C / 4;
    if (C4 < 256 && (256 % C4) != 0) return MCAV_E_INVALID;
    if (C4 > 256 && (C4 % 256) != 0) return MCAV_E_INVALID;
    if (workspace_bytes < mcav_bn_bwd_workspace_bytes(n_pix, C, groups)) return MCAV_E_WORKSPACE;
    const size_t pg = n_pix / groups;
    int blocks = (int)((pg + 31) / 32 < (size_t)BNR_BLOCKS ? (pg + 31) / 32 : (size_t)BNR_BLOCKS);
    float* part = reinterpret_cast<float*>(workspace);
    hipStream_t s = as_stream(stream);
    bn_bwd_reduce_kernel<<<dim3(blocks, groups), 256, 0, s>>>((const f32x4*)dy, (const f32x4*)y_act, (const f32x4*)x, (const f32x4*)save_mean,
                                                              (const f32x4*)save_invstd, relu, pg, C4, part);
    bn_bwd_finalize_kernel<<<(C + 31) / 32, 32 * FIN_SL, 0, s>>>(part, blocks, C, dgamma, dbeta, accumulate, sums, groups);
    return launch_status();
}

MCAV_EXPORT int mcav_bn_bwd_finalize(const float* partial, int nblk, int C, float* dgamma, float* dbeta, int accumulate, float* sums, int groups, void* stream) {
    if (groups < 1) groups = 1;
    if (!partial || !sums || nblk <= 0 || C <= 0) return MCAV_E_INVALID;
    bn_bwd_finalize_kernel<<<(C + 31) / 32, 32 * FIN_SL, 0, as_stream(stream)>>>(partial, nblk, C, dgamma, dbeta, accumulate, sums, groups);
    return launch_status();
}

MCAV_EXPORT int mcav_bn_bwd_apply(const float* dy, const float* y_act, const float* x, const float* gamma, const float* save_mean,
                                  const float* save_invstd, const float* sums, int relu, size_t n_pix, int C, float* dx, float* dres,
                                  int dres_accumulate, int groups, void* stream) {
    if (groups < 1) groups = 1;
    if (!dy || !x || !gamma || !save_mean || !save_invstd || !sums || !dx || C <= 0 || (C & 3) || n_pix == 0 || n_pix % groups) return MCAV_E_INVALID;
    if (relu && !y_act) return MCAV_E_INVALID;
    const size_t n4 = n_pix * (size_t)(C / 4);
    bn_bwd_apply_kernel<<<grid_for(n4), 256, 0, as_stream(stream)>>>((const f32x4*)dy, (const f32x4*)y_act, (const f32x4*)x, (const f32x4*)gamma,
                                                                     (const f32x4*)save_mean, (const f32x4*)save_invstd, (const f32x4*)sums, relu, n4,
                                                                     C / 4, (float)(1.0 / (double)(n_pix / groups)), (f32x4*)dx, (f32x4*)dres, dres_accumulate,
                                                                     (n_pix / groups) * (size_t)(C / 4));
    return launch_status();
}

MCAV_EXPORT int mcav_maxpool3s2_fwd(const float* x, int B, int H, int W, int C, float* y, uint8_t* idx, void* stream) {
    if (!x || !y || !idx || B <= 0 || H <= 0 || W <= 0 || C <= 0 || (C & 3)) return MCAV_E_INVALID;
    const int Ho = (H - 1) / 2 + 1, Wo = (W - 1) / 2 + 1;
    maxpool_fwd_kernel<<<grid_for((size_t)B * Ho * Wo * (C / 4)), 256, 0, as_stream(stream)>>>(x, B, H, W, C, Ho, Wo, y, idx);
    return launch_status();
}

MCAV_EXPORT int mcav_maxpool3s2_bwd(const float* dy, const uint8_t* idx, int B, int H, int W, int C, float* dx, int accumulate, void* stream) {
    if (!dy || !idx || !dx || B <= 0 || H <= 0 || W <= 0 || C <= 0 || (C & 3)) return MCAV_E_INVALID;
    const int Ho = (H - 1) / 2 + 1, Wo = (W - 1) / 2 + 1;
    maxpool_bwd_kernel<<<grid_for((size_t)B * H * W * (C / 4)), 256, 0, as_stream(stream)>>>(dy, idx, B, H, W, C, Ho, Wo, dx, accumulate);
    return launch_status();
}

MCAV_EXPORT int mcav_act_bwd(const float* dy, const float* y, int act, size_t n, float* dx, int accumulate, void* stream) {
    if (!dy || !y || !dx) return MCAV_E_INVALID;
    if (n == 0) return MCAV_OK;
    act_bwd_kernel<<<grid_for(n), 256, 0, as_stream(stream)>>>(dy, y, act, n, dx, accumulate);
    return launch_status();
}

MCAV_EXPORT int mcav_act_bwd_strided(const float* dy, const float* y, int act, size_t n, float* dx, int stride, void* stream) {
    if (!dy || !y || !dx || stride < 1) return MCAV_E_INVALID;
    if (n == 0) return MCAV_OK;
    act_bwd_strided_kernel<<<grid_for(n), 256, 0, as_stream(stream)>>>(dy, y, act, n, dx, stride);
    return launch_status();
}

MCAV_EXPORT int mcav_add(const float* a, const float* b, size_t n, float* out, void* stream) {
    if (!a || !b || !out) return MCAV_E_INVALID;
    if (n == 0) return MCAV_OK;
    add_kernel<<<grid_for(n), 256, 0, as_stream(stream)>>>(a, b, n, out);
    return launch_status();
}

MCAV_EXPORT int mcav_spatial_mean(const float* x, int B, int n_pix, int C, float scale, float* out, void* stream) {
    if (!x || !out || B <= 0 || n_pix <= 0 || C <= 0) return MCAV_E_INVALID;
    spatial_mean_kernel<<<(B * C + 63) / 64, 64, 0, as_stream(stream)>>>(x, B, n_pix, C, scale, out);
    return launch_status();
}

MCAV_EXPORT int mcav_spatial_mean_bwd(const float* dout, int B, int n_pix, int C, float scale, float* dx, void* stream) {
    if (!dout || !dx || B <= 0 || n_pix <= 0 || C <= 0) return MCAV_E_INVALID;
    spatial_mean_bwd_kernel<<<grid_for((size_t)B * n_pix * C), 256, 0, as_stream(stream)>>>(dout, B, n_pix, C, scale, dx);
    return launch_status();
}

MCAV_EXPORT int mcav_adam_step(float* param, const float* grad, float* exp_avg, float* exp_avg_sq, size_t n, float lr, float beta1, float beta2,
                               float eps, int step, float grad_scale, void* stream) {
    if (!param || !grad || !exp_avg || !exp_avg_sq || step < 1) return MCAV_E_INVALID;
    if (n == 0) return MCAV_OK;
    const double bc1 = 1.0 - pow((double)beta1, (double)step);
    const double bc2 = 1.0 - pow((double)beta2, (double)step);
// ... 61 lines not shown
```

unsupervised-pseuso-lidar_amd/csrc/warp_loss.hip:

```cpp
#include <stdlib.h>
#include <mutex>
#include <type_traits>
#include <vector>

#include "mcav_common.h"
#include "kernel_timer.h"
#include "warp_math.h"

namespace mcav {

constexpr int TW = 32, TH = 8, HALO = 2, LW = TW + 2 * HALO, LH = TH + 2 * HALO;
constexpr int WL_SUB = 4, WLH = TH * WL_SUB, WL_LH = WLH + 2 * HALO;
constexpr int NACC = 38;
constexpr int SLAB = 40;

struct PrepConst {
    float Kf[9];
    SampleConst sc;
};

struct WLArgs {
    const float *tgt, *ref0, *ref1, *disp_t, *disp_r0, *poses;
    const void* K;
    const float* upstream;
// ... 556 lines not shown
    l.pc_off = o;   o = align_up(o + sizeof(PrepConst) * (size_t)B, 256);
    l.slab_off = o; o = align_up(o + sizeof(float) * SLAB * (size_t)B * rows, 256);
    l.sl_off = o;   o = align_up(o + sizeof(double) * 2 * (size_t)B, 256);
    l.total = o;
    return l;
}

template <auto KERNEL>
inline int resident_slots() {
    static int slots = 0;
    if (slots == 0) {
        int dev = 0, cus = 256, per_cu = 3;
        hipDeviceProp_t prop;
        if (hipGetDevice(&dev) == hipSuccess && hipGetDeviceProperties(&prop, dev) == hipSuccess && prop.multiProcessorCount > 0) cus = prop.multiProcessorCount;
        if (hipOccupancyMaxActiveBlocksPerMultiprocessor(&per_cu, KERNEL, 256, 0) != hipSuccess || per_cu < 1) per_cu = 3;
        (void)hipGetLastError();
        slots = cus * per_cu;
    }
    return slots;
}
template <unsigned MODE> inline int l1_slots() { return resident_slots<warp_loss_l1_kernel<false, MODE>>(); }
template <unsigned MODE> inline int l1_stereo_slots() { return resident_slots<warp_loss_l1_stereo_kernel<MODE>>(); }

inline void l1_grid(int B, int H, int W, int slots, int& G0, int& G1, bool stereo = false) {
    const int ntiles = ((W + TW - 1) / TW) * ((H + T2H - 1) / T2H);
    static const float ratio_mono = [] { const float r = MCAV_KNOB_FLOAT("MCAV_WL_RATIO", 2.0f); return r > 0.05f ? r : 2.0f; }();
    static const float ratio_stereo = [] { const float r = MCAV_KNOB_FLOAT("MCAV_WL_RATIO_STEREO", 2.7f); return r > 0.05f ? r : 2.7f; }();
    const float ratio = stereo ? ratio_stereo : ratio_mono;
    const int per_sample = slots / B > 0 ? slots / B : 1;
    int n0 = (int)((ntiles * (1.0f + 1.0f / ratio) + per_sample - 1) / per_sample);
    if (n0 < 1) n0 = 1;
    for (;; ++n0) {
        int n1 = (int)(ratio * n0 + 0.5f);
        if (n1 < 1) n1 = 1;
        G0 = (ntiles + n0 - 1) / n0;
        G1 = (ntiles + n1 - 1) / n1;
        if ((G0 + G1) * B <= slots || G0 + G1 <= 2) break;
    }
    static const int xcd_align = MCAV_KNOB_INT("MCAV_WL_XCD", 1);
    if (xcd_align && G0 >= 8 && G1 >= 8) {
        int g0 = (G0 + 7) / 8 * 8, g1 = (G1 + 7) / 8 * 8;
        if ((g0 + g1) * B > slots) g1 = G1 / 8 * 8;
        if ((g0 + g1) * B > slots) g0 = G0 / 8 * 8;
        if (g0 >= 8 && g1 >= 8 && g0 <= ntiles && g1 <= ntiles && (g0 + g1) * B <= slots) { G0 = g0; G1 = g1; }
    }
}

inline dim3 pix_grid(int B, int H, int W) { return dim3((W + TW - 1) / TW, (H + TH - 1) / TH, B); }

}

using namespace mcav;

MCAV_EXPORT int mcav_abi_version(void) { return 1; }

MCAV_EXPORT size_t mcav_warp_loss_workspace_bytes(int B, int H, int W) {
    if (B <= 0 || H <= 0 || W <= 0) return 0;
    return ws_layout(B, H, W).total;
}

static std::mutex g_suspect_mu;
static std::vector<void*> g_suspect_ws;
static bool take_suspect(void* ws) {
    std::lock_guard<std::mutex> lk(g_suspect_mu);
    for (size_t i = 0; i < g_suspect_ws.size(); ++i)
        if (g_suspect_ws[i] == ws) { g_suspect_ws.erase(g_suspect_ws.begin() + i); return true; }
    return false;
}
static void mark_suspect(void* ws) {
    std::lock_guard<std::mutex> lk(g_suspect_mu);
    for (void* p : g_suspect_ws) if (p == ws) return;
    g_suspect_ws.push_back(ws);
}

template <unsigned MODE>
static void launch_fused(const WLArgs& a0, hipStream_t s) {
    WLArgs a = a0;
    if (a.flags & MCAV_WL_SSIM) {
        const dim3 wl_grid((a.W + TW - 1) / TW, (a.H + WLH - 1) / WLH, a.B);
        timed_launch(warp_loss_ssim_kernel<false, MODE>, wl_grid, dim3(256), 0, s, a);
    } else {
        l1_grid(a.B, a.H, a.W, l1_slots<MODE>(), a.G0, a.G1);
        timed_launch(warp_loss_l1_kernel<false, MODE>, dim3(a.G0 + a.G1, a.B), dim3(256), 0, s, a);
    }
}

template <unsigned MODE>
static void launch_stereo(const WLStereoArgs& a0, hipStream_t s) {
    WLStereoArgs a = a0;
    if (a.flags & MCAV_WL_SSIM) {
        const dim3 wl_grid((a.W + TW - 1) / TW, (a.H + WLH - 1) / WLH, a.B);
        timed_launch(warp_loss_ssim_stereo_kernel<MODE>, wl_grid, dim3(256), 0, s, a);
    } else {
        l1_grid(a.B, a.H, a.W, l1_stereo_slots<MODE>(), a.G0, a.G1, true);
        timed_launch(warp_loss_l1_stereo_kernel<MODE>, dim3(a.G0 + a.G1, a.B), dim3(256), 0, s, a);
    }
}

static int warp_loss_launch(const float* tgt, const float* ref0, const float* ref1, const float* disp_t, const float* disp_r0,
                            const float* poses, const void* K, int B, int H, int W, unsigned flags, const float* upstream,
                            const float* term_weights, float* losses, float* d_disp_t, float* d_disp_r0, float* d_poses,
                            void* workspace, size_t workspace_bytes, void* stream, float* dbg, unsigned mode = 0,
                            unsigned char* sel = nullptr, const float* stereo = nullptr, const float* baseline = nullptr) {
    if (!tgt || !ref0 || !ref1 || !disp_t || !disp_r0 || !poses || !K || !losses || !d_disp_t || !d_disp_r0 || !d_poses || !workspace)
        return MCAV_E_INVALID;
    if (B <= 0 || H < 3 || W < 3 || B > WL_MAX_B) return MCAV_E_INVALID;
    const WsLayout l = ws_layout(B, H, W);
// ... 209 lines not shown
```

unsupervised-pseuso-lidar_amd/mcav/depthnet.py:

```python
import torch

from . import nn as N


def spec_of(holder, stride, pad, pad_mode, smallc=False):
    s = getattr(holder, "_mcav_spec", None)
    if s is None or s.weight is not holder.weight:
        s = N.ConvSpec(holder.weight, holder.bias, stride, pad, pad_mode, smallc)
        s.mma = getattr(holder, "_mcav_mma", N.DEFAULT_MMA)
        holder._mcav_spec = s
    return s


def hw(t):
    return (t.shape[1], t.shape[2])


def conv_bn(conv, bn, x, stride, pad, train, relu, residual=None, smallc=False, groups=1, apply=True):
    spec = spec_of(conv, stride, pad, N.PAD_ZERO, smallc)
    if train:
        raw, slab = N.conv_fwd(spec, x, stats=True, groups=groups)
        st = N.bn_train_coeffs(bn, slab, raw.shape[0] * raw.shape[1] * raw.shape[2] // groups, groups)
    else:
        raw = N.conv_fwd(spec, x)
        st = N.bn_eval_coeffs(bn)
    return raw, st, N.bn_apply(raw, st, relu, residual) if apply else None


def block_forward(blk, x, stride, train, groups=1):
    sv = {"x": x, "stride": stride}
    sv["r1"], sv["st1"], sv["h1"] = conv_bn(blk.conv1, blk.bn1, x, stride, 1, train, True, groups=groups)
    if blk.downsample is not None:
        sv["rd"], sv["std"], idt = conv_bn(blk.downsample[0], blk.downsample[1], x, stride, 0, train, False, groups=groups)
    else:
        idt = x
    sv["r2"], sv["st2"], sv["out"] = conv_bn(blk.conv2, blk.bn2, sv["h1"], 1, 1, train, True, residual=idt, groups=groups)
    return sv["out"], sv


def block_backward(blk, sv, dout, addend=None, fused_in=None, consumer=None):
    x, stride = sv["x"], sv["stride"]
    c1 = spec_of(blk.conv1, stride, 1, N.PAD_ZERO)
    c2 = spec_of(blk.conv2, 1, 1, N.PAD_ZERO)
    dr2, dz = N.bn_backward(blk.bn2, sv["st2"], dout, sv["out"], sv["r2"], True, want_dres=True, fused=fused_in)
    N.conv_wgrad(c2, sv["h1"], dr2)
    if N.can_fuse_bn_stats(c2) and sv["st1"].mean is not None:
        dh1, slab, mtg = N.conv_dgrad(c2, dr2, hw(sv["h1"]), dact_aux=sv["h1"], dact=N.ACT_RELU, bn_stats=(sv["r1"], sv["st1"]))
        dr1 = N.bn_backward(blk.bn1, sv["st1"], dh1, None, sv["r1"], True, fused=(slab, mtg))
    else:
        dh1 = N.conv_dgrad(c2, dr2, hw(sv["h1"]))
        dr1 = N.bn_backward(blk.bn1, sv["st1"], dh1, sv["h1"], sv["r1"], True)
    N.conv_wgrad(c1, x, dr1)
    out_stats = None
    kw = {}
    if consumer is not None and N.can_fuse_bn_stats(c1) and consumer["st2"].mean is not None:
        kw = dict(dact_aux=consumer["out"], dact=N.ACT_RELU | N.DACT_AFTER_ADDEND, bn_stats=(consumer["r2"], consumer["st2"]))
    if blk.downsample is None:
        if addend is not None:
            dz = N.add(dz, addend)
        res = N.conv_dgrad(c1, dr1, hw(x), addend=dz, **kw)
    else:
        cd = spec_of(blk.downsample[0], stride, 0, N.PAD_ZERO)
        drd = N.bn_backward(blk.downsample[1], sv["std"], dz, None, sv["rd"], False)
        N.conv_wgrad(cd, x, drd)
        dxd = N.conv_dgrad(cd, drd, hw(x), addend=addend)
        res = N.conv_dgrad(c1, dr1, hw(x), addend=dxd, **kw)
    if kw:
        return res[0], (res[1], res[2])
    return res, None


def bottleneck_forward(blk, x, stride, train, groups=1):
    sv = {"x": x, "stride": stride}
    sv["r1"], sv["st1"], sv["h1"] = conv_bn(blk.conv1, blk.bn1, x, 1, 0, train, True, groups=groups)
    sv["r2"], sv["st2"], sv["h2"] = conv_bn(blk.conv2, blk.bn2, sv["h1"], stride, 1, train, True, groups=groups)
# ... 146 lines not shown
```

unsupervised-pseuso-lidar_amd/mcav/nn.py:

```python
import ctypes
import os
import os as _os

import torch

from . import lib as L

c_p, c_i, c_f, c_sz, c_d = L.c_p, L.c_i, L.c_f, L.c_sz, ctypes.c_double

G_DIRECT, G_SMALLC, G_ADJ_REFLECT, G_ADJ_STRIDE2 = 0, 1, 2, 3
PAD_ZERO, PAD_REFLECT = 0, 1
ACT_NONE, ACT_RELU, ACT_ELU, ACT_SIGMOID = 0, 1, 2, 3
DACT_AFTER_ADDEND = 0x100


class IgemmDesc(ctypes.Structure):
    _fields_ = [("x1", c_p), ("x2", c_p), ("B", c_i), ("Hs", c_i), ("Ws", c_i), ("C1", c_i), ("C2", c_i), ("up1", c_i),
                ("w", c_p), ("kh", c_i), ("kw", c_i), ("Np", c_i), ("Kp", c_i),
                ("mode", c_i), ("stride", c_i), ("sign", c_i), ("offset", c_i), ("pad_mode", c_i),
                ("y", c_p), ("Hd", c_i), ("Wd", c_i), ("Cd", c_i), ("n_begin", c_i), ("n_count", c_i), ("y_choff", c_i),
                ("bias", c_p), ("act", c_i), ("dact_aux", c_p), ("dact", c_i), ("addend", c_p), ("pool", c_i), ("stats", c_p),
                ("tile", c_i), ("groups", c_i), ("w_upmerge", c_p), ("mma", c_i), ("w16", c_p),
                ("stats_x", c_p), ("stats_mean", c_p), ("stats_invstd", c_p), ("w_stem", c_p),
                ("x_planar", c_p * 3), ("planar_B", c_i), ("planar_stack", c_i)]


class WgradDesc(ctypes.Structure):
    _fields_ = [("x1", c_p), ("x2", c_p), ("B", c_i), ("Hs", c_i), ("Ws", c_i), ("C1", c_i), ("C2", c_i), ("up1", c_i),
                ("kh", c_i), ("kw", c_i), ("Kp", c_i),
                ("mode", c_i), ("stride", c_i), ("sign", c_i), ("offset", c_i), ("pad_mode", c_i),
                ("dy", c_p), ("Hd", c_i), ("Wd", c_i), ("Cdy", c_i), ("dy_choff", c_i), ("Cout", c_i), ("Cin", c_i),
                ("dw_oihw", c_p), ("accumulate", c_i), ("dbias", c_p), ("tile", c_i), ("upm", c_i), ("Cin_total", c_i), ("ci_offset", c_i),
                ("mma", c_i),
                ("dy_bn_x", c_p), ("dy_bn_gamma", c_p), ("dy_bn_mean", c_p), ("dy_bn_invstd", c_p), ("dy_bn_sums", c_p),
                ("dy_bn_groups", c_i), ("dy_bn_inv_count", c_f),
                ("x_planar", c_p * 3), ("planar_B", c_i), ("planar_stack", c_i)]


class WgradReduceItem(ctypes.Structure):
    _fields_ = [("slab", c_p), ("pre", c_p), ("dw", c_p), ("dbias", c_p), ("elems", ctypes.c_ulonglong)] + \
               [(n, c_i) for n in ("splits", "groups", "per_group", "Ktot", "slabN", "Kp", "taps", "Cout", "Cin", "ci_t", "accumulate", "upm", "cin_total",
                                   "ci_off", "pre_bx", "red_gx", "red_gy", "pre_first", "red_first", "reserved")]


L.register({
    "mcav_wgrad_deferred": (c_i, [ctypes.POINTER(WgradDesc), c_p, c_sz, ctypes.POINTER(WgradReduceItem), c_p]),
    "mcav_wgrad_reduce_plan": (c_i, [ctypes.POINTER(WgradReduceItem), c_i, ctypes.POINTER(c_i), ctypes.POINTER(c_i), ctypes.POINTER(c_sz)]),
    "mcav_wgrad_reduce_multi": (c_i, [c_p, c_i, c_i, c_i, c_sz, c_p]),
    "mcav_igemm_mtiles": (c_i, [ctypes.POINTER(IgemmDesc)]),
    "mcav_igemm": (c_i, [ctypes.POINTER(IgemmDesc), c_p]),
    "mcav_igemm_uses_bf16": (c_i, [ctypes.POINTER(IgemmDesc)]),
    "mcav_wgrad_uses_bf16": (c_i, [ctypes.POINTER(WgradDesc)]),
    "mcav_f32_to_bf16": (c_i, [c_p, c_p, c_sz, c_p]),
    "mcav_f32_to_bf16_planes": (c_i, [c_p, c_p, c_sz, c_p]),
    "mcav_pack_stem_weights": (c_i, [c_p, c_i, c_i, c_p, c_p]),
    "mcav_wgrad_workspace_bytes": (c_sz, [ctypes.POINTER(WgradDesc)]),
    "mcav_wgrad": (c_i, [ctypes.POINTER(WgradDesc), c_p, c_sz, c_p]),
    "mcav_pack_weights": (c_i, [c_p, c_i, c_i, c_i, c_i, c_i, c_p, c_i, c_i, c_p]),
    "mcav_pack_weights_multi": (c_i, [c_p, c_i, c_i, c_p]),
    "mcav_pack_weights_blocks": (c_i, [c_i, c_i, c_i, c_i]),
    "mcav_pack_weights_upmerge": (c_i, [c_p, c_i, c_i, c_i, c_p, c_i, c_p]),
    "mcav_pack_weights_upmerge_adj": (c_i, [c_p, c_i, c_i, c_i, c_p, c_i, c_i, c_p]),
    "mcav_upsample_adj_fold": (c_i, [c_p, c_i, c_i, c_i, c_i, c_p, c_i, c_p, c_p, c_p]),
    "mcav_nchw_to_nhwc": (c_i, [c_p, c_i, c_i, c_i, c_i, c_p, c_i, c_i, c_p]),
    "mcav_nchw3_to_nhwc": (c_i, [c_p, c_p, c_p, c_i, c_i, c_i, c_i, c_p, c_i, c_p]),
    "mcav_nhwc_to_nchw": (c_i, [c_p, c_i, c_i, c_i, c_i, c_i, c_i, c_p, c_p]),
    "mcav_bn_finalize": (c_i, [c_p, c_i, c_i, c_d, c_p, c_p, c_f, c_f] + [c_p] * 6 + [c_i, c_p, c_sz, c_p]),
    "mcav_bn_finalize_workspace_bytes": (c_sz, [c_i, c_i, c_i]),
    "mcav_bn_eval_coeffs": (c_i, [c_p, c_p, c_p, c_p, c_f, c_i, c_p, c_p, c_p]),
    "mcav_bn_apply": (c_i, [c_p, c_p, c_p, c_p, c_i, c_sz, c_i, c_p, c_sz, c_p]),
    "mcav_bn_bwd_workspace_bytes": (c_sz, [c_sz, c_i, c_i]),
    "mcav_bn_bwd_reduce": (c_i, [c_p] * 5 + [c_i, c_sz, c_i, c_p, c_p, c_i, c_p, c_i, c_p, c_sz, c_p]),
    "mcav_bn_bwd_apply": (c_i, [c_p] * 7 + [c_i, c_sz, c_i, c_p, c_p, c_i, c_i, c_p]),
    "mcav_bn_bwd_finalize": (c_i, [c_p, c_i, c_i, c_p, c_p, c_i, c_p, c_i, c_p]),
    "mcav_maxpool3s2_fwd": (c_i, [c_p, c_i, c_i, c_i, c_i, c_p, c_p, c_p]),
    "mcav_maxpool3s2_bwd": (c_i, [c_p, c_p, c_i, c_i, c_i, c_i, c_p, c_i, c_p]),
    "mcav_stem_bn_relu_pool_fwd": (c_i, [c_p, c_p, c_p, c_i, c_i, c_i, c_i, c_i, c_p, c_p, c_p, c_p]),
    "mcav_stem_pool_bn_bwd_reduce": (c_i, [c_p] * 8 + [c_i] * 6 + [c_p, c_p, c_i, c_p, c_p, c_sz, c_p]),
    "mcav_stem_pool_bn_bwd_apply": (c_i, [c_p] * 10 + [c_i] * 5 + [c_p, c_p]),
    "mcav_act_bwd": (c_i, [c_p, c_p, c_i, c_sz, c_p, c_i, c_p]),
    "mcav_act_bwd_strided": (c_i, [c_p, c_p, c_i, c_sz, c_p, c_i, c_p]),
    "mcav_conv3x3r_c1_fwd": (c_i, [c_p, c_i, c_i, c_i, c_i, c_p, c_p, c_i, c_p, c_p]),
    "mcav_conv3x3r_c1_bwd_workspace_bytes": (c_sz, [c_i]),
    "mcav_conv3x3r_c1_bwd": (c_i, [c_p, c_i, c_i, c_i, c_i, c_p, c_p, c_p, c_i, c_i, c_p, c_p, c_p, c_p, c_i, c_p, c_sz, c_p]),
    "mcav_add": (c_i, [c_p, c_p, c_sz, c_p, c_p]),
    "mcav_spatial_mean": (c_i, [c_p, c_i, c_i, c_i, c_f, c_p, c_p]),
    "mcav_spatial_mean_bwd": (c_i, [c_p, c_i, c_i, c_i, c_f, c_p, c_p]),
    "mcav_upsample_nearest2x": (c_i, [c_p, c_sz, c_i, c_i, c_p, c_p]),
    "mcav_upsample_nearest2x_bwd": (c_i, [c_p, c_sz, c_i, c_i, c_p, c_p]),
    "mcav_adam_step": (c_i, [c_p, c_p, c_p, c_p, c_sz, c_f, c_f, c_f, c_f, c_i, c_f, c_p]),
    "mcav_adam_step_dev": (c_i, [c_p, c_p, c_p, c_p, c_sz, c_f, c_f, c_f, c_p, c_p]),
    "mcav_event_create": (c_i, [ctypes.POINTER(c_p)]),
    "mcav_event_destroy": (c_i, [c_p]),
    "mcav_event_record_external": (c_i, [c_p, c_p]),
    "mcav_event_wait_external": (c_i, [c_p, c_p]),
    "mcav_stream_wait_event": (c_i, [c_p, c_p]),
    "mcav_kernel_timer_begin": (c_i, []),
    "mcav_kernel_timer_count": (c_i, []),
    "mcav_kernel_timer_end": (c_i, [c_p, c_i]),
})


def kernel_timer_begin():
    L.check(L.lib().mcav_kernel_timer_begin(), "mcav_kernel_timer_begin")


def kernel_timer_end():
    n = L.lib().mcav_kernel_timer_count()
    buf = (ctypes.c_float * max(1, n))()
    got = L.lib().mcav_kernel_timer_end(buf, n)
    if got < 0:
        L.check(got, "mcav_kernel_timer_end")
    return [float(buf[i]) for i in range(min(n, got))]


PROFILE = None
PROFILE_LOSS = None
PROFILE_TAGS = None


import collections as _collections
ProfileRec = _collections.namedtuple("ProfileRec", "kind flops i0 i1 executed bf16_planes abytes")


class _Timed:

    def __init__(self, kind, flops, tag="", executed=None, bf16_planes=0, abytes=0.0):
# ... 254 lines not shown
        self.images, self.stack, self.cp = images, stack, cp
        Bp, _, H, W = images[0].shape
        self.shape = (Bp * (len(images) if stack == PLANAR_BATCH else 1), H, W, cp)
        self.device, self.is_cuda = images[0].device, images[0].is_cuda

    def numel(self):
        return sum(t.numel() for t in self.images)

    def fill(self, d):
        d.x1 = None
        for i, t in enumerate(self.images):
            d.x_planar[i] = P(t)
        d.planar_B, d.planar_stack = self.images[0].shape[0], self.stack

    def packed(self):
        if self.stack == PLANAR_CHANNELS:
            return nchw3_to_nhwc(self.images[0], self.images[1], self.images[2], self.cp)
        Bp = self.images[0].shape[0]
        x = torch.zeros(self.shape, dtype=torch.float32, device=self.device)
        for i, t in enumerate(self.images):
            nchw_to_nhwc(t, self.cp, x[i * Bp:(i + 1) * Bp])
        return x


def stats_blocks_stem(spec, stats):
    return stats and not spec.smallc


def _weights_for(spec, d, transposed):
    if spec.mma in (MMA_BF16, MMA_SPLIT, MMA_SPLIT_ALL):
        ph = d.x1 or d.x_planar[0]
        d.mma, d.w16, d.w = spec.mma, ph, ph
        if L.lib().mcav_igemm_uses_bf16(ctypes.byref(d)):
            if spec.mma >= MMA_SPLIT:
                w16 = spec.packed_bwd16s() if transposed else spec.packed_fwd16s()
            else:
                w16 = spec.packed_bwd16() if transposed else spec.packed_fwd16()
            d.w16 = d.w = P(w16)
            return
    d.mma, d.w16 = 0, None
    d.w = P(spec.packed_bwd() if transposed else spec.packed_fwd())


def _planes(d):
    return 6 if d.mma >= MMA_SPLIT else 1 if d.mma == MMA_BF16 else 0


def _pipe_tag(d):
    return " [fp32 on split operands: 6 bf16-MFMA plane products]" if d.mma >= MMA_SPLIT else " [bf16 MFMA]" if d.mma == MMA_BF16 else ""


def out_size(n, k, s, p):
    return (n + 2 * p - k) // s + 1


def conv_fwd(spec, x1, x2=None, up1=False, act=ACT_NONE, stats=False, tile=0, groups=1):
    takes_stem = spec.is_stem() and not stats_blocks_stem(spec, stats) and x2 is None and not up1 and not (tile >> 9) & 1
    planar = x1 if isinstance(x1, PlanarImages) else None
    if planar is not None and not takes_stem:
        x1, planar = planar.packed(), None
    B = x1.shape[0]
    Hs, Ws = (x1.shape[1] * 2, x1.shape[2] * 2) if up1 else (x1.shape[1], x1.shape[2])
    C1 = x1.shape[3]
    C2 = x2.shape[3] if x2 is not None else 0
    Hd, Wd = out_size(Hs, spec.kh, spec.stride, spec.pad), out_size(Ws, spec.kw, spec.stride, spec.pad)
    y = empty((B, Hd, Wd, spec.cout), x1)
    d = IgemmDesc()
    if planar is not None:
        planar.fill(d)
        LAUNCHES["fwd_planar"] += 1
    else:
        d.x1 = P(x1)
    d.x2 = P(x2)
    d.B, d.Hs, d.Ws, d.C1, d.C2, d.up1 = B, Hs, Ws, C1, C2, int(up1)
    d.kh, d.kw, d.Np, d.Kp = spec.kh, spec.kw, spec.np, spec.kp
    d.mode = G_SMALLC if spec.smallc else G_DIRECT
    d.stride, d.sign, d.offset, d.pad_mode = spec.stride, 1, -spec.pad, spec.pad_mode
    d.y, d.Hd, d.Wd, d.Cd, d.n_begin, d.n_count, d.y_choff = P(y), Hd, Wd, spec.cout, 0, spec.cout, 0
    d.bias, d.act = P(spec.bias), act
    d.tile = tile
    d.groups = groups if stats else 1
    _weights_for(spec, d, False)
    if takes_stem:
        d.w_stem = P(spec.packed_stem())
        if spec.mma == MMA_SPLIT_ALL and spec.smallc and spec.cout == 64:
            d.mma = spec.mma
    if (up1 and x2 is not None and not stats and spec.kh == 3 and spec.kw == 3 and spec.stride == 1 and spec.pad == 1
            and spec.pad_mode == PAD_REFLECT and C1 % 16 == 0 and not (tile >> 11) & 1 and not d.mma):
        d.w_upmerge = P(spec.packed_upmerge(C1))
    h = L.lib()
    slab = None
    if stats:
        mt = h.mcav_igemm_mtiles(ctypes.byref(d))
        if mt <= 0:
            raise L.MCAVError("mcav_igemm_mtiles: invalid descriptor (%d)" % mt)
        slab = empty((mt, 2, spec.cout), x1)
        d.stats = P(slab)
    flops = 2.0 * B * Hd * Wd * spec.cout * spec.cin * spec.kh * spec.kw
    executed = flops
    if d.w_upmerge or (up1 and x2 is None and spec.kh == 3 and spec.pad_mode == PAD_REFLECT and C1 in (16, 32) and spec.cout <= 32
                       and not (tile >> 10) & 1 and not (tile >> 9) & 1):
        executed = flops * ((4.0 / 9.0) * C1 + C2) / (C1 + C2)
    if d.w_stem:
        executed = flops * (8.0 / 7.0) * (1.0 if spec.cout >= 32 else 2.0)
    abytes = 4.0 * (x1.numel() + (x2.numel() if x2 is not None else 0) + y.numel() + spec.weight.numel())
    with _Timed("fwd", flops, "M=%d N=%d K=%dx%d s%d %dx%d%s" % (B * Hd * Wd, spec.cout, spec.cin, spec.kh * spec.kw, spec.stride, Hd, Wd, _pipe_tag(d)),
                executed, _planes(d), abytes):
        L.check(h.mcav_igemm(ctypes.byref(d), L.stream()), "mcav_igemm(fwd)")
    return (y, slab) if stats else y


BN_BWD_FUSE = _os.environ.get("MCAV_BN_BWD_FUSE", "1") != "0"


def can_fuse_bn_stats(spec):
    return BN_BWD_FUSE and spec.stride == 1 and spec.pad_mode == PAD_ZERO


def conv_dgrad(spec, dy, in_shape, n_begin=0, n_count=None, out=None, dact_aux=None, dact=ACT_NONE, addend=None, pool=False, tile=0, bn_stats=None):
    B, Hd, Wd, Cout = dy.shape
    Hs, Ws = in_shape
    if n_count is None:
        n_count = spec.cin
    if (pool and n_begin == 0 and out is None and spec.kh == 3 and spec.kw == 3 and spec.stride == 1 and spec.pad == 1
            and spec.pad_mode == PAD_REFLECT and n_count % 16 == 0 and n_count >= UPMERGE_ADJ_MIN_N and Cout == up16(spec.cout)
            and Cout % 32 == 0 and Hs % 2 == 0 and Ws % 2 == 0 and not (tile >> 12) & 1):
        return _dgrad_upsample_merged(spec, dy, (Hs, Ws), n_count, dact_aux, dact, addend, tile)
    y = out if out is not None else empty((B, Hs // 2 if pool else Hs, Ws // 2 if pool else Ws, n_count), dy)
    d = IgemmDesc()
    d.x1, d.x2 = P(dy), None
    d.B, d.Hs, d.Ws, d.C1, d.C2, d.up1 = B, Hd, Wd, Cout, 0, 0
    d.kh, d.kw, d.Np, d.Kp = spec.kh, spec.kw, up16(spec.cin), up16(spec.cout)
    if spec.stride == 1:
        if spec.pad_mode == PAD_REFLECT:
            d.mode, d.stride, d.sign, d.offset = G_ADJ_REFLECT, 1, -1, 1
        else:
            d.mode, d.stride, d.sign, d.offset = G_DIRECT, 1, -1, spec.pad
    elif spec.stride == 2 and spec.pad_mode == PAD_ZERO:
        d.mode, d.stride, d.sign, d.offset = G_ADJ_STRIDE2, 2, -1, spec.pad
    else:
        raise L.MCAVError("conv_dgrad: unsupported stride/padding combination")
    d.pad_mode = PAD_ZERO
    d.y, d.Hd, d.Wd, d.Cd, d.n_begin, d.n_count, d.y_choff = P(y), Hs, Ws, y.shape[3], n_begin, n_count, 0
    d.bias, d.act = None, ACT_NONE
    d.dact_aux, d.dact, d.addend, d.pool = P(dact_aux), dact, P(addend), int(pool)
    d.tile = tile
    _weights_for(spec, d, True)
    slab = None
    if bn_stats is not None:
        x_raw, st = bn_stats
        if pool or n_begin != 0 or n_count != y.shape[3] or tuple(x_raw.shape) != tuple(y.shape) or st.mean is None:
            raise L.MCAVError("conv_dgrad: bn_stats needs an un-pooled, whole-width gradient of the BatchNorm input's shape")
        d.groups = st.groups
        d.stats_x, d.stats_mean, d.stats_invstd = P(x_raw), P(st.mean), P(st.invstd)
        d.stats = d.x1
        mt = L.lib().mcav_igemm_mtiles(ctypes.byref(d))
        if mt <= 0 or mt % st.groups:
            raise L.MCAVError("mcav_igemm_mtiles: invalid descriptor (%d)" % mt)
        slab = empty((mt, 2, n_count), dy)
        d.stats = P(slab)
    with _Timed("dgrad", 2.0 * B * Hd * Wd * spec.cout * n_count * spec.kh * spec.kw,
                "M=%d N=%d K=%dx%d s%d mode%d pool%d %dx%d%s%s" % (B * Hs * Ws, n_count, Cout, spec.kh * spec.kw, spec.stride, d.mode, int(pool), Hs, Ws,
                                                                  " +bn-bwd stats" if slab is not None else "", _pipe_tag(d)), None, _planes(d),
                4.0 * (B * Hd * Wd * spec.cout + y.numel() * (1 + (dact_aux is not None) + (addend is not None) + (slab is not None))
                       + spec.cout * n_count * spec.kh * spec.kw)):
        L.check(L.lib().mcav_igemm(ctypes.byref(d), L.stream()), "mcav_igemm(dgrad)")
    return y if slab is None else (y, slab, slab.shape[0] // bn_stats[1].groups)


UPMERGE_ADJ_MIN_N = int(_os.environ.get("MCAV_UPMERGE_ADJ_MIN_N", "32"))


def _dgrad_upsample_merged(spec, dy, in_shape, c1, dact_aux, dact, addend, tile):
    B, Hd, Wd, Cout = dy.shape
    Hl, Wl = in_shape[0] // 2, in_shape[1] // 2
    tmp = empty((B, Hl + 2, Wl + 2, c1), dy)
    d = IgemmDesc()
    d.x1, d.x2 = P(dy), None
    d.B, d.Hs, d.Ws, d.C1, d.C2, d.up1 = B, Hd, Wd, Cout, 0, 0
    d.kh, d.kw, d.Np, d.Kp = 4, 4, up16(c1), up16(spec.cout)
    d.mode, d.stride, d.sign, d.offset, d.pad_mode = G_DIRECT, 2, 1, -3, PAD_ZERO
    d.y, d.Hd, d.Wd, d.Cd, d.n_begin, d.n_count, d.y_choff = P(tmp), Hl + 2, Wl + 2, c1, 0, c1, 0
    d.bias, d.act = None, ACT_NONE
    d.tile = tile & 0xff
    d.w = P(spec.packed_upmerge_adj(c1))
    if spec.mma in (MMA_BF16, MMA_SPLIT, MMA_SPLIT_ALL):
        d.mma, d.w16 = spec.mma, d.w
        if L.lib().mcav_igemm_uses_bf16(ctypes.byref(d)):
            d.w16 = P(spec.packed_upmerge_adj(c1, bf16=3 if spec.mma >= MMA_SPLIT else True))
        else:
            d.mma, d.w16 = 0, None
    with _Timed("dgrad", 2.0 * B * Hd * Wd * spec.cout * c1 * 9,
                "M=%d N=%d K=%dx9 s1 mode2 pool1 (merged 4x4/s2) %dx%d" % (B * Hd * Wd, c1, Cout, Hd, Wd),
                2.0 * B * (Hl + 2) * (Wl + 2) * spec.cout * c1 * 16, _planes(d),
                4.0 * (dy.numel() + B * Hl * Wl * c1 * (1 + (dact_aux is not None) + (addend is not None)) + spec.cout * c1 * 9)):
        L.check(L.lib().mcav_igemm(ctypes.byref(d), L.stream()), "mcav_igemm(dgrad, merged upsample)")
        y = empty((B, Hl, Wl, c1), dy)
        L.check(L.lib().mcav_upsample_adj_fold(P(tmp), B, Hl, Wl, c1, P(dact_aux), dact, P(addend), P(y), L.stream()), "mcav_upsample_adj_fold")
    return y


LAUNCHES = _collections.Counter()


class DyBn(_collections.namedtuple("DyBn", "x gamma mean invstd sums groups")):
    """conv_wgrad(dy_bn=...): dy is the masked gradient at a train-mode BatchNorm's output and the launch applies the BatchNorm's backward formula
    to it as it loads it (mcav_wgrad_desc.dy_bn_*).  x: the raw conv output; sums: [groups][2][C] of mcav_bn_bwd_finalize."""


def conv_wgrad(spec, x1, dy, x2=None, up1=False, tile=0, dy_bn=None):
    planar = x1 if isinstance(x1, PlanarImages) else None
    if planar is not None and not (spec.is_stem() and x2 is None and not up1 and not (tile >> 9) & 1):
        x1, planar = planar.packed(), None
    B = x1.shape[0]
    Hs, Ws = (x1.shape[1] * 2, x1.shape[2] * 2) if up1 else (x1.shape[1], x1.shape[2])
    gw = grad_buffer(spec.weight)
    gb = grad_buffer(spec.bias) if spec.bias is not None else None
    d = WgradDesc()
    if planar is not None:
        planar.fill(d)
        LAUNCHES["wgrad_planar"] += 1
    else:
        d.x1 = P(x1)
    d.x2 = P(x2)
    d.B, d.Hs, d.Ws, d.C1, d.C2, d.up1 = B, Hs, Ws, x1.shape[3], (x2.shape[3] if x2 is not None else 0), int(up1)
    d.kh, d.kw, d.Kp = spec.kh, spec.kw, spec.kp
    d.mode = G_SMALLC if spec.smallc else G_DIRECT
    d.stride, d.sign, d.offset, d.pad_mode = spec.stride, 1, -spec.pad, spec.pad_mode
    d.dy, d.Hd, d.Wd, d.Cdy, d.dy_choff = P(dy), dy.shape[1], dy.shape[2], dy.shape[3], 0
    d.Cout, d.Cin = spec.cout, spec.cin
    d.dw_oihw, d.accumulate, d.dbias = P(gw), 1, P(gb)
    d.tile = tile
    d.mma = MMA_SPLIT_ALL if (spec.mma == MMA_SPLIT and SPLIT_WGRAD) else (spec.mma if spec.mma in (MMA_BF16, MMA_SPLIT, MMA_SPLIT_ALL) else 0)
    keep = ()
    if dy_bn is not None:
        if dy_bn.x.shape != dy.shape or x2 is not None or up1:
            raise L.MCAVError("conv_wgrad: dy_bn needs the raw conv output in dy's layout and a single source")
        d.dy_bn_x, d.dy_bn_gamma, d.dy_bn_mean, d.dy_bn_invstd, d.dy_bn_sums = P(dy_bn.x), P(dy_bn.gamma), P(dy_bn.mean), P(dy_bn.invstd), P(dy_bn.sums)
        d.dy_bn_groups = dy_bn.groups
        d.dy_bn_inv_count = 1.0 / (B * dy.shape[1] * dy.shape[2] // dy_bn.groups)
        keep = (dy_bn.x, dy_bn.gamma, dy_bn.mean, dy_bn.invstd, dy_bn.sums)
        LAUNCHES["wgrad_dy_bn"] += 1
    bf16 = bool(d.mma and L.lib().mcav_wgrad_uses_bf16(ctypes.byref(d)))
    flops = 2.0 * B * dy.shape[1] * dy.shape[2] * spec.cout * spec.cin * spec.kh * spec.kw
    tag = "pix=%d Cout=%d Ktot=%dx%d s%d" % (B * dy.shape[1] * dy.shape[2], spec.cout, spec.cin, spec.kh * spec.kw, spec.stride)
    c1 = x1.shape[3]
    if bf16 and x2 is not None and c1 % 16 == 0 and x2.shape[3] % 16 == 0:
        c2 = x2.shape[3]
        d.x1, d.x2, d.C1, d.C2, d.up1, d.Kp = P(x2), None, c2, 0, 0, c2
        d.Cin, d.Cin_total, d.ci_offset, d.upm = c2, spec.cin, c1, 0
        launch_wgrad(d, (x2, dy), flops * c2 / spec.cin, tag + " [second source, bf16]")
        d.x1, d.C1, d.up1, d.Kp = P(x1), c1, int(up1), c1
        d.Cin, d.ci_offset, d.dbias = c1, 0, None
        launch_wgrad(d, (x1, dy), flops * c1 / spec.cin, tag + " [first source, bf16]")
        return
# ... 161 lines not shown
        raise L.MCAVError("mcav_wgrad: invalid descriptor")

    dev = tensors[0].device
    planes = _planes(d) if (d.mma and h.mcav_wgrad_uses_bf16(ctypes.byref(d))) else 0
    global LAST_WGRAD_PLANES
    LAST_WGRAD_PLANES = planes
    if planes:
        tag += _pipe_tag(d)
    defer = WGRAD_BATCH.enabled and dev.type == "cuda" and WGRAD_SIDE._note(torch.cuda.current_stream())
    if defer:
        target = (d.dw_oihw, d.ci_offset)
        if target in WGRAD_BATCH.targets:
            flush_wgrad_batch()
        WGRAD_BATCH.targets.add(target)
        ws = WGRAD_BATCH.buffer(nbytes, dev)
        item = WgradReduceItem()
        dd = WgradDesc.from_buffer_copy(d)

        def go_deferred():
            with _Timed("wgrad", flops, tag, executed, planes, abytes):
                L.check(h.mcav_wgrad_deferred(ctypes.byref(dd), P(ws), ws.numel(), ctypes.byref(item), L.stream()), "mcav_wgrad_deferred")
        WGRAD_SIDE.run(go_deferred, tensors)
        WGRAD_BATCH.items.append(item)
        return

    def go():
        ws = L.workspace(nbytes, dev, "wgrad")
        with _Timed("wgrad", flops, tag, executed, planes, abytes):
            L.check(h.mcav_wgrad(ctypes.byref(d), P(ws), ws.numel(), L.stream()), "mcav_wgrad")
    WGRAD_SIDE.run(go, tensors)


def grad_buffer(param):
    if param.grad is None:
        make = getattr(param, "_mcav_grad_view", None)
        param.grad = make() if make is not None else torch.zeros_like(param)
    return param.grad


class BNState:
    __slots__ = ("scale", "shift", "mean", "invstd", "groups")


def bn_train_coeffs(bn, slab, count, groups=1):
    C = bn.weight.shape[0]
    st = BNState()
    buf = empty((4, groups, C), bn.weight)
    st.scale, st.shift, st.mean, st.invstd = buf[0], buf[1], buf[2], buf[3]
    st.groups = groups
    h = L.lib()
    mtiles = slab.shape[0] // groups
    nbytes = h.mcav_bn_finalize_workspace_bytes(mtiles, C, groups)
    ws = L.workspace(nbytes, slab.device, "bn_fin", zero=True) if nbytes else None
    L.check(h.mcav_bn_finalize(P(slab), mtiles, C, float(count), P(bn.weight), P(bn.bias), bn.eps, bn.momentum,
                               P(bn.running_mean), P(bn.running_var), P(st.scale), P(st.shift), P(st.mean), P(st.invstd), groups,
                               P(ws), ws.numel() if ws is not None else 0, L.stream()), "mcav_bn_finalize")
    _NBT_PENDING.append((bn.num_batches_tracked, groups))
    if len(_NBT_PENDING) >= 256:
        flush_bn_counters()
    return st


_NBT_PENDING = []


def flush_bn_counters():
    if _NBT_PENDING:
        by_inc = {}
        for t, inc in _NBT_PENDING:
            by_inc.setdefault(inc, []).append(t)
        for inc, ts in by_inc.items():
            torch._foreach_add_(ts, inc)
        _NBT_PENDING.clear()


def bn_eval_coeffs(bn):
    C = bn.weight.shape[0]
    st = BNState()
    buf = empty((2, C), bn.weight)
    st.scale, st.shift, st.mean, st.invstd = buf[0], buf[1], None, None
    st.groups = 1
    L.check(L.lib().mcav_bn_eval_coeffs(P(bn.weight), P(bn.bias), P(bn.running_mean), P(bn.running_var), bn.eps, C, P(st.scale), P(st.shift),
                                        L.stream()), "mcav_bn_eval_coeffs")
    return st


def bn_apply(x, st, relu, residual=None):
    y = torch.empty_like(x)
    C = x.shape[-1]
    n_pix = x.numel() // C
    L.check(L.lib().mcav_bn_apply(P(x), P(st.scale), P(st.shift), P(residual), ACT_RELU if relu else ACT_NONE, n_pix, C, P(y),
                                  n_pix // st.groups, L.stream()), "mcav_bn_apply")
    return y


def bn_backward(bn, st, dy, y_act, x, relu, want_dres=False, dres_out=None, dres_accumulate=False, fused=None):
    C = x.shape[-1]
    n_pix = x.numel() // C
    h = L.lib()
    G = st.groups
    if fused is not None:
        slab, mtg = fused
        sums = empty((G, 2, C), x)
        gg, gb = grad_buffer(bn.weight), grad_buffer(bn.bias)
        L.check(h.mcav_bn_bwd_finalize(P(slab), mtg, C, P(gg), P(gb), 1, P(sums), G, L.stream()), "mcav_bn_bwd_finalize")
        dx = torch.empty_like(x)
        L.check(h.mcav_bn_bwd_apply(P(dy), None, P(x), P(bn.weight), P(st.mean), P(st.invstd), P(sums), 0, n_pix, C, P(dx), None, 0, G, L.stream()),
                "mcav_bn_bwd_apply")
        if want_dres:
            if dres_out is not None:
                raise L.MCAVError("bn_backward: a fused gradient is its own residual gradient (no dres_out)")
            return dx, dy
        return dx
    ws = L.workspace(h.mcav_bn_bwd_workspace_bytes(n_pix, C, G), x.device, "bn_bwd")
    sums = empty((G, 2, C), x)
    gg, gb = grad_buffer(bn.weight), grad_buffer(bn.bias)
    L.check(h.mcav_bn_bwd_reduce(P(dy), P(y_act), P(x), P(st.mean), P(st.invstd), int(relu), n_pix, C, P(gg), P(gb), 1, P(sums), G, P(ws),
                                 ws.numel(), L.stream()), "mcav_bn_bwd_reduce")
    dx = torch.empty_like(x)
    dres = None
    if want_dres:
        dres = dres_out if dres_out is not None else torch.empty_like(x)
    L.check(h.mcav_bn_bwd_apply(P(dy), P(y_act), P(x), P(bn.weight), P(st.mean), P(st.invstd), P(sums), int(relu), n_pix, C, P(dx), P(dres),
                                int(dres_accumulate), G, L.stream()), "mcav_bn_bwd_apply")
    return (dx, dres) if want_dres else dx


def nchw_to_nhwc(src, Cp, dst=None, choff=0):
    B, C, H, W = src.shape
    if dst is None:
        dst = torch.zeros((B, H, W, Cp), dtype=torch.float32, device=src.device)
    L.check(L.lib().mcav_nchw_to_nhwc(P(src), B, C, H, W, P(dst), Cp, choff, L.stream()), "mcav_nchw_to_nhwc")
    return dst


def nchw3_to_nhwc(s0, s1, s2, Cp):
    B, C, H, W = s0.shape
    if s1.shape != s0.shape or s2.shape != s0.shape:
        raise L.MCAVError("nchw3_to_nhwc: the three images must have one shape")
    dst = torch.empty((B, H, W, Cp), dtype=torch.float32, device=s0.device)
    L.check(L.lib().mcav_nchw3_to_nhwc(P(s0), P(s1), P(s2), B, C, H, W, P(dst), Cp, L.stream()), "mcav_nchw3_to_nhwc")
    return dst


def nhwc_to_nchw(src, C=None, choff=0):
    B, H, W, Cp = src.shape
    C = Cp if C is None else C
    dst = empty((B, C, H, W), src)
    L.check(L.lib().mcav_nhwc_to_nchw(P(src), B, C, H, W, Cp, choff, P(dst), L.stream()), "mcav_nhwc_to_nchw")
    return dst


def maxpool_fwd(x):
    B, H, W, C = x.shape
    Ho, Wo = (H - 1) // 2 + 1, (W - 1) // 2 + 1
    y = empty((B, Ho, Wo, C), x)
    idx = torch.empty((B, Ho, Wo, C), dtype=torch.uint8, device=x.device)
    L.check(L.lib().mcav_maxpool3s2_fwd(P(x), B, H, W, C, P(y), P(idx), L.stream()), "mcav_maxpool3s2_fwd")
    return y, idx


# ... 119 lines not shown
```

Before: 1148 images/s.

## Fold BN stats finalize into apply via ticketed in-epilogue pre-reduction

Conv epilogues now optionally pre-reduce the per-tile BN stat rows into fp64 partial rows, using an atomic ticket so that the last tile of each row group does the sum. A new bn_apply_train kernel then finishes the mean/var from those few rows and applies scale/shift/residual/relu in one launch, replacing the separate bn_finalize and bn_apply launches. It is on by default for the forward pass. A matching fused backward path is added but gated off by default. In exchange the last tile of each group does extra serialized work and atomics, and every apply block re-reduces the row sums redundantly.

```diff
diff --git a/include/mcav_conv.h b/include/mcav_conv.h
--- a/include/mcav_conv.h
+++ b/include/mcav_conv.h
@@ -52,9 +52,13 @@
     const float* x_planar[3];
     int planar_B;
     int planar_stack;
+    double* stats_pre;
+    unsigned* stats_tickets;
+    int stats_rows;
 } mcav_igemm_desc;
 
 int mcav_igemm_mtiles(const mcav_igemm_desc* d);
+int mcav_igemm_stats_rows(int tiles_per_group);
 int mcav_igemm(const mcav_igemm_desc* d, void* stream);
 int mcav_igemm_uses_bf16(const mcav_igemm_desc* d);
 
@@ -147,6 +151,14 @@
                       const float* save_invstd, const float* sums, int relu, size_t n_pix, int C, float* dx, float* dres,
                       int dres_accumulate, int groups, void* stream);
 
+int mcav_bn_apply_train(const float* x, const void* rows, int rows_f64, int nrows, int C, double count, const float* gamma, const float* beta,
+                        float eps, float momentum, float* running_mean, float* running_var, float* scale, float* shift, float* save_mean,
+                        float* save_invstd, int groups, const float* residual, int act, size_t n_pix, float* y, void* stream);
+int mcav_bn_bwd_apply_fused(const float* dy, const float* y_act, const float* x, const float* gamma, const float* save_mean,
+                            const float* save_invstd, const void* rows, int rows_f64, int nrows, int relu, size_t n_pix, int C,
+                            float* dgamma, float* dbeta, int accumulate, float* sums, float* dx, float* dres, int dres_accumulate,
+                            int groups, void* stream);
+
 int mcav_maxpool3s2_fwd(const float* x, int B, int H, int W, int C, float* y, uint8_t* idx, void* stream);
 int mcav_maxpool3s2_bwd(const float* dy, const uint8_t* idx, int B, int H, int W, int C, float* dx, int accumulate, void* stream);
 
diff --git a/unsupervised-pseuso-lidar_amd/csrc/conv_bf16.hip b/unsupervised-pseuso-lidar_amd/csrc/conv_bf16.hip
--- a/unsupervised-pseuso-lidar_amd/csrc/conv_bf16.hip
+++ b/unsupervised-pseuso-lidar_amd/csrc/conv_bf16.hip
@@ -338,7 +338,7 @@
 #pragma unroll
             for (int j = 0; j < T::TN; ++j) acc[i][j] += mid[i][j] + low[i][j];
     }
-    igemm_epilogue_lean<T>(p, acc, s_out, s_stat, tid, wm0, wn0, n0, mt);
+    igemm_epilogue_lean<T, !REFL>(p, acc, s_out, s_stat, tid, wm0, wn0, n0, mt);
 }
 
 __device__ __forceinline__ int patch_pixel(int R) {
@@ -621,7 +621,7 @@
         for (int t = 0; t < TMB; ++t) acc[t][0] += mid[t] + low[t];
     }
     if (diag & 16) return;
-    igemm_epilogue_lean<T>(p, acc, s_out, s_stat, tid, wm0, wn0, n0, mt);
+    igemm_epilogue_lean<T, !ADJ>(p, acc, s_out, s_stat, tid, wm0, wn0, n0, mt);
 }
 
 template <int NS, int TMB>
@@ -862,7 +862,7 @@
     }
     if constexpr (NS > 1) acc[0][0] += mid + low;
     if (diag & 16) return;
-    igemm_epilogue_lean<T>(p, acc, s_out, s_stat, tid, wm0, wn0, n0, mt);
+    igemm_epilogue_lean<T, !ADJ>(p, acc, s_out, s_stat, tid, wm0, wn0, n0, mt);
 }
 
 #ifndef MCAV_PATCH2_DIAG
diff --git a/unsupervised-pseuso-lidar_amd/csrc/conv_gather.h b/unsupervised-pseuso-lidar_amd/csrc/conv_gather.h
--- a/unsupervised-pseuso-lidar_amd/csrc/conv_gather.h
+++ b/unsupervised-pseuso-lidar_amd/csrc/conv_gather.h
@@ -99,6 +99,9 @@
     int pool;
     float* stats;
     const float *stats_x, *stats_mean, *stats_invstd;
+    double* stats_pre;
+    unsigned* stats_tickets;
+    int stats_rows;
     int M;
     int Mc, McP;
     int groups;
diff --git a/unsupervised-pseuso-lidar_amd/csrc/conv_igemm.hip b/unsupervised-pseuso-lidar_amd/csrc/conv_igemm.hip
--- a/unsupervised-pseuso-lidar_amd/csrc/conv_igemm.hip
+++ b/unsupervised-pseuso-lidar_amd/csrc/conv_igemm.hip
@@ -291,7 +291,7 @@
         __builtin_amdgcn_sched_barrier(0);
         __syncthreads();
     }
-    igemm_epilogue<T>(p, acc, s_out, s_stat, tid, wm0, wn0, n0, mt);
+    igemm_epilogue<T, KIND != K_REFLADJ && stats_pre_tile<T>()>(p, acc, s_out, s_stat, tid, wm0, wn0, n0, mt);
 }
 
 
@@ -761,9 +761,9 @@
         IgemmParams q = p;
         q.y = p.kslab + (size_t)ks * ((size_t)p.g.B * p.Hd * p.Wd * p.Cd);
         q.bias = nullptr; q.act = MCAV_ACT_NONE; q.dact_aux = nullptr; q.addend = nullptr; q.stats = nullptr; q.stats_x = nullptr;
-        igemm_epilogue_lean<T>(q, acc, s_out, s_stat, tid, wm0, wn0, n0, mt);
+        igemm_epilogue_lean<T, false>(q, acc, s_out, s_stat, tid, wm0, wn0, n0, mt);
     } else {
-        igemm_epilogue_lean<T>(p, acc, s_out, s_stat, tid, wm0, wn0, n0, mt);
+        igemm_epilogue_lean<T, TK == 0 && stats_pre_tile<T>()>(p, acc, s_out, s_stat, tid, wm0, wn0, n0, mt);
     }
     MCAV_STAMP(5);
 }
@@ -1656,6 +1656,8 @@
     p.bias = d->bias; p.act = d->act; p.dact_aux = d->dact_aux; p.dact = d->dact; p.addend = d->addend; p.pool = d->pool; p.stats = d->stats;
     if (d->stats_x && (!d->stats || !d->stats_mean || !d->stats_invstd || d->pool || d->y_choff != 0 || d->n_begin != 0 || d->n_count != d->Cd)) return false;
     p.stats_x = d->stats ? d->stats_x : nullptr; p.stats_mean = d->stats_mean; p.stats_invstd = d->stats_invstd;
+    if (d->stats_pre && (!d->stats || !d->stats_tickets || d->stats_rows < 1)) return false;
+    p.stats_pre = d->stats_pre; p.stats_tickets = d->stats_tickets; p.stats_rows = d->stats_rows;
     const long Mlin = (long)d->B * d->Hd * d->Wd;
     if ((long)d->B * d->Hs * d->Ws * (d->C1 > d->C2 ? d->C1 : d->C2) * 4 >= 0x7fffffffL) return false;
     if ((long)d->Np * kstride_of(d->kh * d->kw, d->Kp) * 4 >= 0x7fffffffL) return false;
@@ -1803,6 +1805,11 @@
     return p.mtiles;
 }
 
+MCAV_EXPORT int mcav_igemm_stats_rows(int tiles_per_group) {
+    if (tiles_per_group <= 64) return 0;
+    return round_up((tiles_per_group + 63) / 64, 8);
+}
+
 bool mcav_try_halo(const mcav_igemm_desc* d, hipStream_t s);
 int mcav_bf16_igemm(const mcav_igemm_desc* d, hipStream_t s);
 bool mcav_try_stem(const mcav_igemm_desc* d, const mcav::IgemmParams& p, hipStream_t s);
@@ -1820,6 +1827,13 @@
     if (planar) { dp = *d; if (!dp.x1) dp.x1 = d->x_planar[0]; d = &dp; }
     if (!fill_params(d, p, tile)) return MCAV_E_INVALID;
     hipStream_t s = as_stream(stream);
+    if (d->stats_pre) {
+        const int mt = mcav_igemm_mtiles(d), g = p.groups;
+        int bm, bn;
+        tile_dims(tile, bm, bn);
+        if (bn < 32) return MCAV_E_INVALID;
+        if (planar || d->mode != MCAV_G_DIRECT || mt <= 0 || mt % g != 0 || mcav_stem_mtiles(d) || d->stats_rows != mcav_igemm_stats_rows(mt / g)) return MCAV_E_INVALID;
+    }
     if (planar) return mcav_try_stem(d, p, s) ? launch_status() : MCAV_E_INVALID;
     if (mcav_try_halo(d, s)) return launch_status();
     if (mcav_try_stem(d, p, s)) return launch_status();
diff --git a/unsupervised-pseuso-lidar_amd/csrc/conv_shared.h b/unsupervised-pseuso-lidar_amd/csrc/conv_shared.h
--- a/unsupervised-pseuso-lidar_amd/csrc/conv_shared.h
+++ b/unsupervised-pseuso-lidar_amd/csrc/conv_shared.h
@@ -94,7 +94,41 @@
 
 enum { K_FAST = 0, K_REFLADJ = 1, K_GENERIC = 2 };
 
-template <class T>
+template <class T> constexpr bool stats_pre_tile() { return T::BN >= 32; }
+template <int BN>
+__device__ __forceinline__ void stats_prereduce(const IgemmParams& p, float* s_word, int tid, int n0, int mt) {
+    handoff_release();
+    __syncthreads();
+    const int tpg = p.mtiles / p.groups, grp = mt / tpg, tin = mt - grp * tpg;
+    const int rg = tin / p.stats_rows, nrg = (tpg + p.stats_rows - 1) / p.stats_rows;
+    const int first = rg * p.stats_rows, cnt = min(p.stats_rows, tpg - first);
+    unsigned* tk = p.stats_tickets + ((size_t)(grp * nrg + rg) * p.ntiles + n0 / BN);
+    int* s_last = reinterpret_cast<int*>(s_word);
+    if (tid == 0) *s_last = handoff_ticket(tk) == (unsigned)(cnt - 1);
+    __syncthreads();
+    if (!*s_last) return;
+    const size_t rstride = (size_t)2 * p.n_count;
+    for (int e = tid; e < 2 * BN; e += 256) {
+        const int which = e / BN, col = e - which * BN;
+        if (n0 + col < p.n_count) {
+            const float* src = p.stats + ((size_t)(grp * tpg + first) * 2 + which) * p.n_count + n0 + col;
+            double s = 0.0;
+            int r = 0;
+            for (; r + 8 <= cnt; r += 8) {
+                float v[8];
+#pragma unroll
+                for (int u = 0; u < 8; ++u) v[u] = handoff_load(src + (size_t)(r + u) * rstride);
+#pragma unroll
+                for (int u = 0; u < 8; ++u) s += (double)v[u];
+            }
+            for (; r < cnt; ++r) s += (double)handoff_load(src + (size_t)r * rstride);
+            p.stats_pre[((size_t)(grp * nrg + rg) * 2 + which) * p.n_count + n0 + col] = s;
+        }
+    }
+    if (tid == 0) handoff_store(tk, 0u);
+}
+
+template <class T, bool kPre = true>
 __device__ __forceinline__ void igemm_epilogue(const IgemmParams& p, typename T::AccT (&acc)[T::TM][T::TN], const int* s_out,
                                                float (*s_stat)[2][T::BN], int tid, int wm0, int wn0, int n0, int mt) {
     constexpr int BN = T::BN;
@@ -172,13 +206,16 @@
                 float s = 0.f;
 #pragma unroll
                 for (int wmi = 0; wmi < T::WAVES_M; ++wmi) s += s_stat[wmi][which][col];
-                p.stats[((size_t)mt * 2 + which) * p.n_count + n0 + col] = s;
-            }
-        }
-    }
-}
-
-template <class T>
+                float* o = &p.stats[((size_t)mt * 2 + which) * p.n_count + n0 + col];
+                if (kPre && p.stats_pre) handoff_store(o, s);
+                else *o = s;
+            }
+        }
+        if (kPre && p.stats_pre) stats_prereduce<BN>(p, &s_stat[0][0][0], tid, n0, mt);
+    }
+}
+
+template <class T, bool kPre = true>
 __device__ __forceinline__ void igemm_epilogue_lean(const IgemmParams& p, typename T::AccT (&acc)[T::TM][T::TN], const unsigned* s_outb,
                                                     float (*s_stat)[2][T::BN], int tid, int wm0, int wn0, int n0, int mt) {
     constexpr int BN = T::BN, MF = T::MF, NQ = T::ACC / 4;
@@ -299,9 +336,12 @@
                 float s = 0.f;
 #pragma unroll
                 for (int wmi = 0; wmi < T::WAVES_M; ++wmi) s += s_stat[wmi][which][col];
-                p.stats[((size_t)mt * 2 + which) * p.n_count + n0 + col] = s;
-            }
-        }
+                float* o = &p.stats[((size_t)mt * 2 + which) * p.n_count + n0 + col];
+                if (kPre && p.stats_pre) handoff_store(o, s);
+                else *o = s;
+            }
+        }
+        if (kPre && p.stats_pre) stats_prereduce<BN>(p, &s_stat[0][0][0], tid, n0, mt);
     }
 }
 
diff --git a/unsupervised-pseuso-lidar_amd/csrc/conv_stem.hip b/unsupervised-pseuso-lidar_amd/csrc/conv_stem.hip
--- a/unsupervised-pseuso-lidar_amd/csrc/conv_stem.hip
+++ b/unsupervised-pseuso-lidar_amd/csrc/conv_stem.hip
@@ -238,7 +238,7 @@
         });
         __syncthreads();
         if constexpr (kWide) stem_epilogue_wide<E>(p, acc, s_out, s_stat, tid, wave * TM * 32, mt);
-        else igemm_epilogue_lean<E>(p, acc, s_out, s_stat, tid, wave * TM * 32, 0, 0, mt);
+        else igemm_epilogue_lean<E, false>(p, acc, s_out, s_stat, tid, wave * TM * 32, 0, 0, mt);
     }
 }
 
@@ -394,7 +394,7 @@
 #pragma unroll
             for (int j = 0; j < TN; ++j) acc[i][j] += mid[i][j] + low[i][j];
         __syncthreads();
-        if (!(SS_DIAG & 2)) igemm_epilogue_lean<E>(p, acc, s_out, s_stat, tid, wave * TM * 32, 0, 0, mt);
+        if (!(SS_DIAG & 2)) igemm_epilogue_lean<E, false>(p, acc, s_out, s_stat, tid, wave * TM * 32, 0, 0, mt);
     }
 }
 
diff --git a/unsupervised-pseuso-lidar_amd/csrc/nn_ops.hip b/unsupervised-pseuso-lidar_amd/csrc/nn_ops.hip
--- a/unsupervised-pseuso-lidar_amd/csrc/nn_ops.hip
+++ b/unsupervised-pseuso-lidar_amd/csrc/nn_ops.hip
@@ -338,6 +338,152 @@
         f32x4 gi, t2;
         bn_bwd_dx_coeffs(gamma[c], is, sg[C4 + c], inv_count, gi, t2);
         dx[i] = bn_bwd_dx(g, x[i], mean[grp * C4 + c], is, gi, sg[c], inv_count, t2);
+    }
+}
+
+template <class TIn>
+__device__ __forceinline__ double bn_rows_sum(const TIn* src, int nrows, size_t stride) {
+    double s = 0.0;
+    int r = 0;
+    for (; r + 8 <= nrows; r += 8) {
+        TIn v[8];
+#pragma unroll
+        for (int u = 0; u < 8; ++u) v[u] = src[(size_t)(r + u) * stride];
+#pragma unroll
+        for (int u = 0; u < 8; ++u) s += (double)v[u];
+    }
+    for (; r < nrows; ++r) s += (double)src[(size_t)r * stride];
+    return s;
+}
+
+template <class TIn>
+__global__ __launch_bounds__(256) void bn_apply_train_kernel(const f32x4* x, const TIn* rows, int nrows, int C, double count, const float* gamma,
+                                                             const float* beta, float eps, float momentum, float* running_mean, float* running_var,
+                                                             float* scale, float* shift, float* save_mean, float* save_invstd, const f32x4* res,
+                                                             int relu, size_t ppg, f32x4* y) {
+    __shared__ double s_sum[2][64];
+    __shared__ __attribute__((aligned(16))) float s_sc[64], s_sh[64];
+    const int tid = threadIdx.x, cq = tid & 15, pl = tid >> 4;
+    const int c0 = blockIdx.x * 64, g = blockIdx.z, groups = gridDim.z, C4 = C >> 2;
+    const size_t per = (ppg + gridDim.y - 1) / gridDim.y, p0 = blockIdx.y * per, p1 = p0 + per < ppg ? p0 + per : ppg;
+    const size_t base = (size_t)g * ppg * C4 + (c0 >> 2) + cq;
+    size_t pix = p0 + pl;
+    f32x4 xv = {0.f, 0.f, 0.f, 0.f}, rv = {0.f, 0.f, 0.f, 0.f};
+    if (pix < p1) {
+        xv = x[base + pix * C4];
+        if (res) rv = res[base + pix * C4];
+    }
+    const bool owner = blockIdx.y == 0 && g == 0;
+    const int g_end = owner ? groups : g + 1;
+    for (int gg = g; gg < g_end; ++gg) {
+        if (tid < 128) {
+            const int which = tid >> 6, col = tid & 63;
+            s_sum[which][col] = bn_rows_sum(rows + ((size_t)gg * nrows * 2 + which) * C + c0 + col, nrows, (size_t)2 * C);
+        }
+        __syncthreads();
+        if (tid < 64) {
+            const int c = c0 + tid;
+            const double mean = s_sum[0][tid] / count;
+            double var = s_sum[1][tid] / count - mean * mean;
+            if (var < 0.0) var = 0.0;
+            const float invstd = (float)(1.0 / sqrt(var + (double)eps));
+            const float sc = gamma[c] * invstd;
+            const float sh = beta[c] - (float)mean * sc;
+            if (gg == g) { s_sc[tid] = sc; s_sh[tid] = sh; }
+            if (owner) {
+                scale[gg * C + c] = sc;
+                shift[gg * C + c] = sh;
+                save_mean[gg * C + c] = (float)mean;
+                save_invstd[gg * C + c] = invstd;
+                if (running_mean) {
+                    const double unbiased = count > 1.0 ? var * count / (count - 1.0) : var;
+                    running_mean[c] = (1.0f - momentum) * running_mean[c] + momentum * (float)mean;
+                    running_var[c] = (1.0f - momentum) * running_var[c] + momentum * (float)unbiased;
+                }
+            }
+        }
+        __syncthreads();
+    }
+    const f32x4 sc = *reinterpret_cast<const f32x4*>(&s_sc[cq * 4]), sh = *reinterpret_cast<const f32x4*>(&s_sh[cq * 4]);
+    while (pix < p1) {
+        const size_t nx = pix + 16;
+        f32x4 xn = {0.f, 0.f, 0.f, 0.f}, rn = {0.f, 0.f, 0.f, 0.f};
+        if (nx < p1) {
+            xn = x[base + nx * C4];
+            if (res) rn = res[base + nx * C4];
+        }
+        f32x4 v = xv * sc + sh;
+        if (res) v += rv;
+        if (relu) { v.x = fmaxf(v.x, 0.f); v.y = fmaxf(v.y, 0.f); v.z = fmaxf(v.z, 0.f); v.w = fmaxf(v.w, 0.f); }
+        y[base + pix * C4] = v;
+        xv = xn; rv = rn; pix = nx;
+    }
+}
+
+template <class TIn>
+__global__ __launch_bounds__(256) void bn_bwd_apply_fused_kernel(const f32x4* dy, const f32x4* yact, const f32x4* x, const float* gamma, const float* mean,
+                                                                 const float* invstd, const TIn* rows, int nrows, int relu, size_t ppg, int C,
+                                                                 float inv_count, float* dgamma, float* dbeta, int accumulate, float* sums, f32x4* dx,
+                                                                 f32x4* dres, int dres_acc) {
+    __shared__ double s_sum[2][64];
+    __shared__ __attribute__((aligned(16))) float s_s1[64], s_s2[64];
+    const int tid = threadIdx.x, cq = tid & 15, pl = tid >> 4;
+    const int c0 = blockIdx.x * 64, g = blockIdx.z, groups = gridDim.z, C4 = C >> 2;
+    const size_t per = (ppg + gridDim.y - 1) / gridDim.y, p0 = blockIdx.y * per, p1 = p0 + per < ppg ? p0 + per : ppg;
+    const size_t base = (size_t)g * ppg * C4 + (c0 >> 2) + cq;
+    size_t pix = p0 + pl;
+    const f32x4 z = {0.f, 0.f, 0.f, 0.f};
+    f32x4 gv = z, xv = z, ya = z, dr = z;
+    if (pix < p1) {
+        gv = dy[base + pix * C4];
+        xv = x[base + pix * C4];
+        if (relu) ya = yact[base + pix * C4];
+        if (dres && dres_acc) dr = dres[base + pix * C4];
+    }
+    const bool owner = blockIdx.y == 0 && g == 0;
+    const int g_end = owner ? groups : g + 1;
+    double ta = 0.0, tb = 0.0;
+    for (int gg = g; gg < g_end; ++gg) {
+        if (tid < 128) {
+            const int which = tid >> 6, col = tid & 63;
+            s_sum[which][col] = bn_rows_sum(rows + ((size_t)gg * nrows * 2 + which) * C + c0 + col, nrows, (size_t)2 * C);
+        }
+        __syncthreads();
+        if (tid < 64) {
+            const int c = c0 + tid;
+            const double a = s_sum[0][tid], b = s_sum[1][tid];
+            if (gg == g) { s_s1[tid] = (float)a; s_s2[tid] = (float)b; }
+            if (owner) {
+                sums[(size_t)gg * 2 * C + c] = (float)a;
+                sums[(size_t)gg * 2 * C + C + c] = (float)b;
+                ta += a; tb += b;
+            }
+        }
+        __syncthreads();
+    }
+    if (owner && tid < 64) {
+        const int c = c0 + tid;
+        if (dbeta) dbeta[c] = accumulate ? dbeta[c] + (float)ta : (float)ta;
+        if (dgamma) dgamma[c] = accumulate ? dgamma[c] + (float)tb : (float)tb;
+    }
+    const int cg = g * C4 + (c0 >> 2) + cq;
+    const f32x4 mu = reinterpret_cast<const f32x4*>(mean)[cg], is = reinterpret_cast<const f32x4*>(invstd)[cg];
+    const f32x4 s1 = *reinterpret_cast<const f32x4*>(&s_s1[cq * 4]);
+    f32x4 gi, t2;
+    bn_bwd_dx_coeffs(reinterpret_cast<const f32x4*>(gamma)[(c0 >> 2) + cq], is, *reinterpret_cast<const f32x4*>(&s_s2[cq * 4]), inv_count, gi, t2);
+    while (pix < p1) {
+        const size_t nx = pix + 16;
+        f32x4 gn = z, xn = z, yn = z, dn = z;
+        if (nx < p1) {
+            gn = dy[base + nx * C4];
+            xn = x[base + nx * C4];
+            if (relu) yn = yact[base + nx * C4];
+            if (dres && dres_acc) dn = dres[base + nx * C4];
+        }
+        if (relu) gv = relu_mask(gv, ya);
+        if (dres) dres[base + pix * C4] = dres_acc ? dr + gv : gv;
+        dx[base + pix * C4] = bn_bwd_dx(gv, xv, mu, is, gi, s1, inv_count, t2);
+        gv = gn; xv = xn; ya = yn; dr = dn; pix = nx;
     }
 }
 
@@ -604,6 +750,58 @@
     return launch_status();
 }
 
+static dim3 bn_fused_grid(int C, size_t ppg, int groups) {
+    const int cols = C / 64;
+    size_t slices = (ppg + 15) / 16;
+    size_t cap = 2048 / ((size_t)cols * groups);
+    if (cap < 1) cap = 1;
+    if (slices > cap) slices = cap;
+    return dim3(cols, (unsigned)slices, groups);
+}
+
+MCAV_EXPORT int mcav_bn_apply_train(const float* x, const void* rows, int rows_f64, int nrows, int C, double count, const float* gamma, const float* beta,
+                                    float eps, float momentum, float* running_mean, float* running_var, float* scale, float* shift, float* save_mean,
+                                    float* save_invstd, int groups, const float* residual, int act, size_t n_pix, float* y, void* stream) {
+    if (groups < 1) groups = 1;
+    if (!x || !rows || !gamma || !beta || !scale || !shift || !save_mean || !save_invstd || !y || count <= 0) return MCAV_E_INVALID;
+    if (nrows <= 0 || nrows > BNF_DIRECT || C <= 0 || (C & 63) || groups > 65535 || (act != MCAV_ACT_NONE && act != MCAV_ACT_RELU)) return MCAV_E_INVALID;
+    if ((running_mean == nullptr) != (running_var == nullptr) || n_pix == 0 || n_pix % groups) return MCAV_E_INVALID;
+    const size_t ppg = n_pix / groups;
+    const dim3 grid = bn_fused_grid(C, ppg, groups);
+    hipStream_t s = as_stream(stream);
+    if (rows_f64)
+        bn_apply_train_kernel<double><<<grid, 256, 0, s>>>((const f32x4*)x, (const double*)rows, nrows, C, count, gamma, beta, eps, momentum, running_mean,
+                                                           running_var, scale, shift, save_mean, save_invstd, (const f32x4*)residual,
+                                                           act == MCAV_ACT_RELU, ppg, (f32x4*)y);
+    else
+        bn_apply_train_kernel<float><<<grid, 256, 0, s>>>((const f32x4*)x, (const float*)rows, nrows, C, count, gamma, beta, eps, momentum, running_mean,
+                                                          running_var, scale, shift, save_mean, save_invstd, (const f32x4*)residual,
+                                                          act == MCAV_ACT_RELU, ppg, (f32x4*)y);
+    return launch_status();
+}
+
+MCAV_EXPORT int mcav_bn_bwd_apply_fused(const float* dy, const float* y_act, const float* x, const float* gamma, const float* save_mean,
+                                        const float* save_invstd, const void* rows, int rows_f64, int nrows, int relu, size_t n_pix, int C,
+                                        float* dgamma, float* dbeta, int accumulate, float* sums, float* dx, float* dres, int dres_accumulate,
+                                        int groups, void* stream) {
+    if (groups < 1) groups = 1;
+    if (!dy || !x || !gamma || !save_mean || !save_invstd || !rows || !sums || !dx || n_pix == 0 || n_pix % groups) return MCAV_E_INVALID;
+    if (nrows <= 0 || nrows > BNF_DIRECT || C <= 0 || (C & 63) || groups > 65535 || (relu && !y_act)) return MCAV_E_INVALID;
+    const size_t ppg = n_pix / groups;
+    const dim3 grid = bn_fused_grid(C, ppg, groups);
+    const float inv_count = (float)(1.0 / (double)ppg);
+    hipStream_t s = as_stream(stream);
+    if (rows_f64)
+        bn_bwd_apply_fused_kernel<double><<<grid, 256, 0, s>>>((const f32x4*)dy, (const f32x4*)y_act, (const f32x4*)x, gamma, save_mean, save_invstd,
+                                                               (const double*)rows, nrows, relu, ppg, C, inv_count, dgamma, dbeta, accumulate, sums,
+                                                               (f32x4*)dx, (f32x4*)dres, dres_accumulate);
+    else
+        bn_bwd_apply_fused_kernel<float><<<grid, 256, 0, s>>>((const f32x4*)dy, (const f32x4*)y_act, (const f32x4*)x, gamma, save_mean, save_invstd,
+                                                              (const float*)rows, nrows, relu, ppg, C, inv_count, dgamma, dbeta, accumulate, sums,
+                                                              (f32x4*)dx, (f32x4*)dres, dres_accumulate);
+    return launch_status();
+}
+
 MCAV_EXPORT int mcav_maxpool3s2_fwd(const float* x, int B, int H, int W, int C, float* y, uint8_t* idx, void* stream) {
     if (!x || !y || !idx || B <= 0 || H <= 0 || W <= 0 || C <= 0 || (C & 3)) return MCAV_E_INVALID;
     const int Ho = (H - 1) / 2 + 1, Wo = (W - 1) / 2 + 1;
diff --git a/unsupervised-pseuso-lidar_amd/csrc/warp_loss.hip b/unsupervised-pseuso-lidar_amd/csrc/warp_loss.hip
--- a/unsupervised-pseuso-lidar_amd/csrc/warp_loss.hip
+++ b/unsupervised-pseuso-lidar_amd/csrc/warp_loss.hip
@@ -632,7 +632,7 @@
 
 using namespace mcav;
 
-MCAV_EXPORT int mcav_abi_version(void) { return 1; }
+MCAV_EXPORT int mcav_abi_version(void) { return 2; }
 
 MCAV_EXPORT size_t mcav_warp_loss_workspace_bytes(int B, int H, int W) {
     if (B <= 0 || H <= 0 || W <= 0) return 0;
diff --git a/unsupervised-pseuso-lidar_amd/mcav/depthnet.py b/unsupervised-pseuso-lidar_amd/mcav/depthnet.py
--- a/unsupervised-pseuso-lidar_amd/mcav/depthnet.py
+++ b/unsupervised-pseuso-lidar_amd/mcav/depthnet.py
@@ -20,7 +20,11 @@
     spec = spec_of(conv, stride, pad, N.PAD_ZERO, smallc)
     if train:
         raw, slab = N.conv_fwd(spec, x, stats=True, groups=groups)
-        st = N.bn_train_coeffs(bn, slab, raw.shape[0] * raw.shape[1] * raw.shape[2] // groups, groups)
+        count = raw.shape[0] * raw.shape[1] * raw.shape[2] // groups
+        if apply:
+            st, y = N.bn_train_apply(bn, slab, count, groups, raw, relu, residual)
+            return raw, st, y
+        st = N.bn_train_coeffs(bn, slab, count, groups)
     else:
         raw = N.conv_fwd(spec, x)
         st = N.bn_eval_coeffs(bn)
diff --git a/unsupervised-pseuso-lidar_amd/mcav/nn.py b/unsupervised-pseuso-lidar_amd/mcav/nn.py
--- a/unsupervised-pseuso-lidar_amd/mcav/nn.py
+++ b/unsupervised-pseuso-lidar_amd/mcav/nn.py
@@ -22,7 +22,8 @@
                 ("bias", c_p), ("act", c_i), ("dact_aux", c_p), ("dact", c_i), ("addend", c_p), ("pool", c_i), ("stats", c_p),
                 ("tile", c_i), ("groups", c_i), ("w_upmerge", c_p), ("mma", c_i), ("w16", c_p),
                 ("stats_x", c_p), ("stats_mean", c_p), ("stats_invstd", c_p), ("w_stem", c_p),
-                ("x_planar", c_p * 3), ("planar_B", c_i), ("planar_stack", c_i)]
+                ("x_planar", c_p * 3), ("planar_B", c_i), ("planar_stack", c_i),
+                ("stats_pre", c_p), ("stats_tickets", c_p), ("stats_rows", c_i)]
 
 
 class WgradDesc(ctypes.Structure):
@@ -48,6 +49,7 @@
     "mcav_wgrad_reduce_plan": (c_i, [ctypes.POINTER(WgradReduceItem), c_i, ctypes.POINTER(c_i), ctypes.POINTER(c_i), ctypes.POINTER(c_sz)]),
     "mcav_wgrad_reduce_multi": (c_i, [c_p, c_i, c_i, c_i, c_sz, c_p]),
     "mcav_igemm_mtiles": (c_i, [ctypes.POINTER(IgemmDesc)]),
+    "mcav_igemm_stats_rows": (c_i, [c_i]),
     "mcav_igemm": (c_i, [ctypes.POINTER(IgemmDesc), c_p]),
     "mcav_igemm_uses_bf16": (c_i, [ctypes.POINTER(IgemmDesc)]),
     "mcav_wgrad_uses_bf16": (c_i, [ctypes.POINTER(WgradDesc)]),
@@ -73,6 +75,8 @@
     "mcav_bn_bwd_reduce": (c_i, [c_p] * 5 + [c_i, c_sz, c_i, c_p, c_p, c_i, c_p, c_i, c_p, c_sz, c_p]),
     "mcav_bn_bwd_apply": (c_i, [c_p] * 7 + [c_i, c_sz, c_i, c_p, c_p, c_i, c_i, c_p]),
     "mcav_bn_bwd_finalize": (c_i, [c_p, c_i, c_i, c_p, c_p, c_i, c_p, c_i, c_p]),
+    "mcav_bn_apply_train": (c_i, [c_p, c_p, c_i, c_i, c_i, c_d, c_p, c_p, c_f, c_f] + [c_p] * 6 + [c_i, c_p, c_i, c_sz, c_p, c_p]),
+    "mcav_bn_bwd_apply_fused": (c_i, [c_p] * 7 + [c_i, c_i, c_i, c_sz, c_i, c_p, c_p, c_i, c_p, c_p, c_p, c_i, c_i, c_p]),
     "mcav_maxpool3s2_fwd": (c_i, [c_p, c_i, c_i, c_i, c_i, c_p, c_p, c_p]),
     "mcav_maxpool3s2_bwd": (c_i, [c_p, c_p, c_i, c_i, c_i, c_i, c_p, c_i, c_p]),
     "mcav_stem_bn_relu_pool_fwd": (c_i, [c_p, c_p, c_p, c_i, c_i, c_i, c_i, c_i, c_p, c_p, c_p, c_p]),
@@ -433,6 +437,28 @@
 
 def out_size(n, k, s, p):
     return (n + 2 * p - k) // s + 1
+
+
+BN_FOLD_FWD = _os.environ.get("MCAV_BN_FOLD_FWD", "1") != "0"
+BN_FOLD_BWD = _os.environ.get("MCAV_BN_FOLD_BWD", "0") != "0"
+
+StatRows = _collections.namedtuple("StatRows", "rows f64 nrows")
+
+
+def _stats_second_level(d, slab, mt, groups, n_count):
+    groups = max(1, groups)
+    if n_count % 64 or mt % groups or (d.tile & 0xff) in (4, 6):
+        return
+    tpg = mt // groups
+    rows = L.lib().mcav_igemm_stats_rows(tpg)
+    if rows == 0:
+        slab.fold_rows = StatRows(None, 0, tpg)
+        return
+    nrg = -(-tpg // rows)
+    pre = torch.empty((groups, nrg, 2, n_count), dtype=torch.float64, device=slab.device)
+    tickets = L.workspace(max(4 * groups * 64 * ((n_count + 15) // 16), 1 << 17), slab.device, "bn_fold_tickets", zero=True)
+    d.stats_pre, d.stats_tickets, d.stats_rows = P(pre), P(tickets), rows
+    slab.fold_rows = StatRows(pre, 1, nrg)
 
 
 def conv_fwd(spec, x1, x2=None, up1=False, act=ACT_NONE, stats=False, tile=0, groups=1):
@@ -477,6 +503,8 @@
             raise L.MCAVError("mcav_igemm_mtiles: invalid descriptor (%d)" % mt)
         slab = empty((mt, 2, spec.cout), x1)
         d.stats = P(slab)
+        if BN_FOLD_FWD and not takes_stem and not spec.smallc:
+            _stats_second_level(d, slab, mt, d.groups, spec.cout)
     flops = 2.0 * B * Hd * Wd * spec.cout * spec.cin * spec.kh * spec.kw
     executed = flops
     if d.w_upmerge or (up1 and x2 is None and spec.kh == 3 and spec.pad_mode == PAD_REFLECT and C1 in (16, 32) and spec.cout <= 32
@@ -540,6 +568,8 @@
             raise L.MCAVError("mcav_igemm_mtiles: invalid descriptor (%d)" % mt)
         slab = empty((mt, 2, n_count), dy)
         d.stats = P(slab)
+        if BN_FOLD_BWD:
+            _stats_second_level(d, slab, mt, st.groups, n_count)
     with _Timed("dgrad", 2.0 * B * Hd * Wd * spec.cout * n_count * spec.kh * spec.kw,
                 "M=%d N=%d K=%dx%d s%d mode%d pool%d %dx%d%s%s" % (B * Hs * Ws, n_count, Cout, spec.kh * spec.kw, spec.stride, d.mode, int(pool), Hs, Ws,
                                                                   " +bn-bwd stats" if slab is not None else "", _pipe_tag(d)), None, _planes(d),
@@ -582,6 +612,7 @@
 
 
 LAUNCHES = _collections.Counter()
+BN_LAUNCHES = _collections.Counter()
 
 
 class DyBn(_collections.namedtuple("DyBn", "x gamma mean invstd sums groups")):
@@ -849,6 +880,7 @@
     mtiles = slab.shape[0] // groups
     nbytes = h.mcav_bn_finalize_workspace_bytes(mtiles, C, groups)
     ws = L.workspace(nbytes, slab.device, "bn_fin", zero=True) if nbytes else None
+    BN_LAUNCHES["bn_finalize"] += 1
     L.check(h.mcav_bn_finalize(P(slab), mtiles, C, float(count), P(bn.weight), P(bn.bias), bn.eps, bn.momentum,
                                P(bn.running_mean), P(bn.running_var), P(st.scale), P(st.shift), P(st.mean), P(st.invstd), groups,
                                P(ws), ws.numel() if ws is not None else 0, L.stream()), "mcav_bn_finalize")
@@ -869,6 +901,27 @@
         for inc, ts in by_inc.items():
             torch._foreach_add_(ts, inc)
         _NBT_PENDING.clear()
+
+
+def bn_train_apply(bn, slab, count, groups, x, relu, residual=None):
+    fold = getattr(slab, "fold_rows", None) if BN_FOLD_FWD else None
+    if fold is None:
+        st = bn_train_coeffs(bn, slab, count, groups)
+        return st, bn_apply(x, st, relu, residual)
+    C = bn.weight.shape[0]
+    st = BNState()
+    buf = empty((4, groups, C), bn.weight)
+    st.scale, st.shift, st.mean, st.invstd = buf[0], buf[1], buf[2], buf[3]
+    st.groups = groups
+    y = torch.empty_like(x)
+    BN_LAUNCHES["bn_apply_train"] += 1
+    L.check(L.lib().mcav_bn_apply_train(P(x), P(fold.rows if fold.f64 else slab), fold.f64, fold.nrows, C, float(count), P(bn.weight), P(bn.bias), bn.eps, bn.momentum,
+                                        P(bn.running_mean), P(bn.running_var), P(st.scale), P(st.shift), P(st.mean), P(st.invstd), groups,
+                                        P(residual), ACT_RELU if relu else ACT_NONE, x.numel() // C, P(y), L.stream()), "mcav_bn_apply_train")
+    _NBT_PENDING.append((bn.num_batches_tracked, groups))
+    if len(_NBT_PENDING) >= 256:
+        flush_bn_counters()
+    return st, y
 
 
 def bn_eval_coeffs(bn):
@@ -900,10 +953,17 @@
         slab, mtg = fused
         sums = empty((G, 2, C), x)
         gg, gb = grad_buffer(bn.weight), grad_buffer(bn.bias)
-        L.check(h.mcav_bn_bwd_finalize(P(slab), mtg, C, P(gg), P(gb), 1, P(sums), G, L.stream()), "mcav_bn_bwd_finalize")
         dx = torch.empty_like(x)
-        L.check(h.mcav_bn_bwd_apply(P(dy), None, P(x), P(bn.weight), P(st.mean), P(st.invstd), P(sums), 0, n_pix, C, P(dx), None, 0, G, L.stream()),
-                "mcav_bn_bwd_apply")
+        fold = getattr(slab, "fold_rows", None) if BN_FOLD_BWD else None
+        if fold is not None:
+            BN_LAUNCHES["bn_bwd_apply_fused"] += 1
+            L.check(h.mcav_bn_bwd_apply_fused(P(dy), None, P(x), P(bn.weight), P(st.mean), P(st.invstd), P(fold.rows if fold.f64 else slab), fold.f64, fold.nrows, 0, n_pix, C,
+                                              P(gg), P(gb), 1, P(sums), P(dx), None, 0, G, L.stream()), "mcav_bn_bwd_apply_fused")
+        else:
+            BN_LAUNCHES["bn_bwd_finalize"] += 1
+            L.check(h.mcav_bn_bwd_finalize(P(slab), mtg, C, P(gg), P(gb), 1, P(sums), G, L.stream()), "mcav_bn_bwd_finalize")
+            L.check(h.mcav_bn_bwd_apply(P(dy), None, P(x), P(bn.weight), P(st.mean), P(st.invstd), P(sums), 0, n_pix, C, P(dx), None, 0, G, L.stream()),
+                    "mcav_bn_bwd_apply")
         if want_dres:
             if dres_out is not None:
                 raise L.MCAVError("bn_backward: a fused gradient is its own residual gradient (no dres_out)")
```

Measured after the change: 1149 images/s, median of 3. No clear change (+0.1%).
